# XuyangBai/D3Feat

Measured on AMD Instinct MI355X. Metric: fragments/sec (30k-pt clouds), higher is better.
Workload: dtype f32; 1 GPU; SURVEY §8d config #2: synthetic 3DMatch room fragment, 300k raw pts -> grid subsample 0.03 m (~29k pts per cloud) -> self-pair -> 5-level pyramid -> full KPFCNN forward (random-init weights (reference initialiser, seed 42), 14.1M params)...; points_per_cloud=29369, fragments_per_gpu=2141, parallelism=fragment-dp1, fragments_per_replay=12, engine_fallbacks=0, engine_isolated_replays=0

## Files before the change

### d3feat_amd/_lib.py

```python
import ctypes as C
import os

_HERE = os.path.dirname(os.path.abspath(__file__))
LIB_PATH = os.environ.get("D3FEAT_AMD_LIB") or os.path.join(_HERE, "lib", "libd3feat_amd.so")

D3F_OK = 0
ERRORS = {-1: "HIP runtime / kernel launch failure", -2: "workspace too small", -3: "invalid argument"}
ST_EMPTY_ELEMENT, ST_NEG_CELL, ST_KEY_RANGE, ST_HIT_OVERFLOW, ST_OUT_OVERFLOW, ST_KEY_WIDTH = 1, 2, 4, 8, 16, 32
PAD_NUM_SUPPORTS = -2147483648
NEIGHBOR_CAP = 1024
MAX_BATCH = 255
TOPK_MAX = 8192
PAIRS_KMAX = 1024
REPEAT_COUNTS_MAX = 16
MATCH_KMAX = 8192
VALIDATION_NMAX = 1024
SCENES_MAX = 256
GRID_RESET_MAX = 8
VP_INDEX_RANGE, VP_COUNT_RANGE = 1, 2

_vp, _sz, _i, _f = C.c_void_p, C.c_size_t, C.c_int, C.c_float

SIGNATURES = {
    "d3f_version": (_i, []),
    "d3f_trace_marker": (_i, [_i, _vp]),
    "d3f_pack_status": (_i, [_vp, _vp, _i, _vp, _i, _vp, _i, _vp, _i, _vp, _i, _i, _i, _vp]),
    "d3f_grid_subsample_workspace_bytes": (_sz, [_i, _i, _i, _i]),
    "d3f_batch_grid_subsample": (_i, [_vp, _i, _vp, _i, _f, _vp, _i, _vp, _i, _vp, _vp, _vp, _vp, _vp, _vp, _sz, _vp]),
    "d3f_batch_grid_subsample_async": (_i, [_vp, _i, _vp, _i, _f, _vp, _i, _i, _i, _vp, _vp, _vp, _sz, _vp]),
    "d3f_batch_grid_subsample_async_inplace": (_i, [_vp, _i, _vp, _i, _f, _vp, _i, _i, _vp, _vp, _vp, _sz, _vp]),
    "d3f_stack_self_pair": (_i, [_vp, _i, _vp, _i, _vp, _vp, _vp, _vp]),
    "d3f_radius_neighbors_workspace_bytes": (_sz, [_i, _i, _i]),
    "d3f_batch_radius_neighbors": (_i, [_vp, _i, _vp, _i, _vp, _vp, _i, _f, _vp, _i, _i, _i, _vp, _vp, _sz, _vp]),
    "d3f_neighbor_grid_bytes": (_sz, [_i, _i]),
    "d3f_neighbor_grid_order_offset": (_sz, [_i, _i]),
    "d3f_neighbor_grid_build": (_i, [_vp, _i, _vp, _i, _f, _vp, _sz, _vp]),
    "d3f_neighbor_grid_boxed_form": (_i, [_i, _i]),
    "d3f_geometry_reset": (_i, [_vp, _i, _vp, _vp, _vp, _vp, _i, _vp]),
    "d3f_neighbor_grid_build_boxed": (_i, [_vp, _i, _vp, _i, _f, _vp, _vp, _sz, _vp]),
    "d3f_stack_self_pair_boxed": (_i, [_vp, _i, _vp, _i, _vp, _vp, _vp, _vp, _vp, _vp]),
    "d3f_batch_grid_subsample_async_boxed": (_i, [_vp, _vp, _i, _vp, _i, _f, _vp, _i, _i, _i, _vp, _vp, _vp, _vp, _vp, _sz, _vp]),
    "d3f_neighbor_grid_search": (_i, [_vp, _sz, _i, _vp, _i, _vp, _i, _f, _i, _vp, _i, _i, _i, _i, _i, _f, _i, _vp, _vp]),
    "d3f_neighbor_grid_search_ordered": (_i, [_vp, _sz, _i, _vp, _i, _vp, _i, _f, _vp, _sz, _vp, _i, _i, _i, _i, _i, _f, _i, _vp, _vp]),
    "d3f_neighbor_grid_inv_offset": (_sz, [_i, _i]),
    "d3f_neighbor_grid_xyz_offset": (_sz, [_i, _i]),
    "d3f_row_positive": (_i, [_vp, _i, _i, _i, _vp, _vp, _i, _vp]),
    "d3f_kpconv_aggregate": (_i, [_vp, _i, _vp, _i, _vp, _i, _i, _vp, _i, _i, _vp, _vp, _i, _f, _i, _i, _vp, _vp, _vp, _vp,
                                  _vp, _i, _vp]),
    "d3f_kpconv_deform_aggregate": (_i, [_vp, _i, _vp, _i, _vp, _i, _i, _vp, _i, _i, _vp, _i, _f, _vp, _i, _i, _vp, _i, _f, _i, _i, _vp,
                                         _vp, _vp, _vp, _i, _vp]),
    "d3f_kpconv_fused_c1": (_i, [_vp, _i, _vp, _i, _vp, _i, _i, _vp, _i, _vp, _i, _f, _i, _i, _vp, _i, _vp, _vp, _vp, _i, _i,
                                 _f, _vp, _i, _vp, _vp, _vp, _i, _vp]),
    "d3f_kpconv_fused32": (_i, [_vp, _i, _vp, _i, _vp, _i, _i, _vp, _i, _vp, _vp, _i, _f, _i, _i, _vp, _vp, _vp, _vp, _i, _i, _f, _vp,
                                _i, _vp, _vp, _vp, _i, _vp]),
    "d3f_kpconv_fused_supported": (_i, [_i, _i, _i, _i, _i]),
    "d3f_kpconv_pack_weights": (_i, [_vp, _i, _i, _vp, _vp]),
    "d3f_kpconv_fused": (_i, [_vp, _i, _vp, _i, _vp, _i, _i, _vp, _i, _i, _vp, _vp, _i, _f, _i, _i, _vp, _i, _vp, _vp, _vp, _i, _i,
                              _f, _vp, _i, _vp, _vp, _vp, _i, _vp]),
    "d3f_kpconv_fused32_x3": (_i, [_vp, _i, _vp, _i, _vp, _i, _i, _vp, _i, _vp, _vp, _i, _f, _i, _i, _vp, _vp, _vp, _vp, _i, _i, _f, _vp,
                                   _i, _vp, _vp, _vp, _i, _vp]),
    "d3f_kpconv_packed_x3_bytes": (_sz, [_i, _i]),
    "d3f_kpconv_pack_weights_x3": (_i, [_vp, _i, _i, _vp, _vp]),
    "d3f_kpconv_fused_x3": (_i, [_vp, _i, _vp, _i, _vp, _i, _i, _vp, _i, _i, _vp, _vp, _i, _f, _i, _i, _vp, _i, _vp, _vp, _vp, _i, _i,
                                 _f, _vp, _i, _vp, _vp, _vp, _i, _vp]),
    "d3f_gemm_workspace_bytes": (_sz, [_i, _i, _i, _i]),
    "d3f_gemm_bf16_workspace_bytes": (_sz, [_i, _i, _i, _i]),
    "d3f_gemm_f32": (_i, [_vp, _i, _vp, _i, _vp, _i, _i, _i, _i, _vp, _vp, _vp, _vp, _i, _i, _f, _vp, _sz, _vp, _i, _vp]),
    "d3f_gemm_upsample_cat_f32": (_i, [_vp, _i, _i, _i, _vp, _i, _vp, _i, _i, _vp, _i, _vp, _i, _i, _i, _vp, _vp, _i, _f, _vp, _sz,
                                       _vp, _vp, _i, _vp]),
    "d3f_ind_max_pool": (_i, [_vp, _i, _i, _i, _vp, _i, _i, _i, _vp, _i, _vp, _vp, _vp, _vp, _i, _vp]),
    "d3f_closest_pool_cat": (_i, [_vp, _i, _i, _i, _vp, _i, _i, _vp, _i, _i, _vp, _i, _vp, _vp, _vp]),
    "d3f_affine_act": (_i, [_vp, _i, _i, _i, _vp, _vp, _vp, _i, _i, _f, _vp, _i, _vp, _vp]),
    "d3f_pack_descriptors": (_i, [_vp, _vp, _i, _i, _vp, _i, _vp, _i, _vp, _vp]),
    "d3f_pack_descriptors_to": (_i, [_vp, _vp, _i, _i, _vp, _i, _vp, _i, _vp, _vp, _i, _i, _i, _vp, _vp, _vp]),
    "d3f_topk_workspace_bytes": (_sz, [_i, _i, _i, _i]),
    "d3f_topk_records": (_i, [_vp, _i, _vp, _i, _i, _vp, _i, _i, _vp, _vp, _i, _i, _i, _vp, _i, _i, _vp, _i, _vp, _vp, _vp, _vp, _sz,
                              _vp]),
    "d3f_feature_nn_workspace_bytes": (_sz, [_i]),
    "d3f_feature_nn": (_i, [_vp, _i, _i, _vp, _i, _i, _i, _vp, _vp, _vp, _sz, _vp]),
    "d3f_mutual_matches_workspace_bytes": (_sz, [_i]),
    "d3f_mutual_matches": (_i, [_vp, _i, _vp, _i, _vp, _vp, _vp, _sz, _vp]),
    "d3f_ransac_hypotheses": (_i, [_vp, _i, _vp, _i, _vp, _i, _f, _f, C.c_uint64, C.c_uint64, _i, _vp, _vp, _vp]),
    "d3f_ransac_draw": (_i, [C.c_uint64, C.c_uint64, _i, _i]),
    "d3f_neighbor_grid_score": (_i, [_vp, _sz, _i, _vp, _i, _vp, _i, _f, _vp, _vp, _vp, _vp]),
    "d3f_register_pairs_workspace_bytes": (_sz, [_i, _i, _i, _i]),
    "d3f_register_pairs": (_i, [_vp, _i, _i, _i, _i, _vp, _vp, _i, _i, _f, _i, _f, _f, _i, _i, C.c_uint64, _vp, _f] + [_vp] * 11
                           + [_sz, _vp]),
    "d3f_repeatability_pairs": (_i, [_vp, _i, _i, _i, _vp, _vp, _i, _vp, _i, _vp, _vp, _i, _vp, _vp, _vp]),
    "d3f_match_pairs_workspace_bytes": (_sz, [_i, _vp, _i]),
    "d3f_match_pairs": (_i, [_vp, _i, _i, _i, _i, _vp, _vp, _i, _vp, _f, _vp, _i, _vp, _vp, _vp, _sz, _vp]),
    "d3f_register_pairs_counts_workspace_bytes": (_sz, [_i, _i, _i, _vp, _i, _i]),
    "d3f_register_pairs_counts": (_i, [_vp, _i, _i, _i, _i, _vp, _vp, _i, _vp, _i, _f, _i, _f, _f, _i, _i, C.c_uint64, _vp, _f] + [_vp] * 10
                                  + [_sz, _vp]),
    "d3f_overlap_pairs": (_i, [_vp, _sz, _i, _i, _vp, _i, _f, _vp, _vp, _i, _vp]),
    "d3f_validation_pairs_workspace_bytes": (_sz, [_i, _i]),
    "d3f_validation_pairs": (_i, [_vp, _i, _i, _vp, _i, _vp, _i, _i, _vp, _vp, _vp, _i, _vp, _i, _f, _i, _f, _f, _f, _f] + [_vp] * 5
                             + [_sz, _vp]),
    "d3f_loss_gradients_workspace_bytes": (_sz, [_i, _i, _i]),
    "d3f_loss_gradients": (_i, [_vp, _i, _i, _vp, _i, _vp, _i, _i, _vp, _vp, _vp, _i, _vp, _i, _f, _i, _f, _f, _f, _f, _i, _vp, _i, _vp, _i,
                                _vp, _vp, _vp, _sz, _vp]),
    "d3f_neighbor_transpose_workspace_bytes": (_sz, [_i, _i]),
    "d3f_neighbor_transpose": (_i, [_vp, _i, _i, _i, _vp, _i, _vp, _vp, _vp, _sz, _vp]),
    "d3f_detect_head_backward_workspace_bytes": (_sz, [_i, _i, _i]),
    "d3f_detect_head_backward": (_i, [_vp, _i, _i, _i, _vp, _i, _i, _vp, _vp, _i, _i, _vp, _vp, _vp, _i, _vp, _i, _vp, _i, _vp, _sz, _vp]),
    "d3f_neighbor_transpose_qs": (_i, [_vp, _i, _i, _i, _vp, _i, _vp, _vp, _vp, _vp, _sz, _vp]),
    "d3f_kpconv_backward_workspace_bytes": (_sz, [_i, _i, _i, _i, _i, _i]),
    "d3f_kpconv_backward": (_i, [_vp, _i, _vp, _i, _vp, _i, _i, _vp, _i, _i, _vp, _i, _f, _i, _i, _vp, _vp, _i, _i, _vp, _vp, _vp, _i, _vp,
                                 _vp, _vp, _vp, _i, _vp, _sz, _vp]),
    "d3f_gemm_tn_workspace_bytes": (_sz, [_i, _i, _i]),
    "d3f_gemm_tn_f32": (_i, [_vp, _i, _vp, _i, _i, _i, _i, _vp, _vp, _vp, _sz, _vp]),
    "d3f_batch_norm_workspace_bytes": (_sz, [_i, _i]),
    "d3f_batch_norm_train": (_i, [_vp, _i, _i, _i, _vp, _vp, _f, _f, _vp, _vp, _vp, _i, _i, _f, _vp, _i, _vp, _vp, _vp, _vp, _sz, _vp]),
    "d3f_batch_norm_backward": (_i, [_vp, _i, _vp, _i, _vp, _i, _i, _i, _vp, _vp, _vp, _i, _f, _vp, _i, _vp, _vp, _vp, _i, _vp, _vp, _sz,
                                     _vp]),
    "d3f_pose_errors": (_i, [_vp, _vp, _i, _i, _vp, _vp, _vp, _vp, _vp, _vp]),
    "d3f_sanitize_descriptors": (_i, [_vp, _i, _i, _i, _i, _vp]),
    "d3f_matching_summary": (_i, [_vp, _vp, _vp, _i, _i, _vp, _i, _vp, _vp, _vp, _vp]),
    "d3f_registration_recall": (_i, [_vp, _i, _vp, _vp, _vp, _vp, _vp, _i, _i, _vp, _i, _vp, _vp, _vp, _vp, _vp]),
    "d3f_icp_pairs_workspace_bytes": (_sz, [_i, _i]),
    "d3f_icp_pairs": (_i, [_vp, _sz, _i, _vp, _i, _vp, _i, _vp, _vp, _i, _i] + [_vp] * 9 + [_sz, _vp]),
    "d3f_gemm_pack_bf16": (_i, [_vp, _i, _i, _i, _vp, _vp]),
    "d3f_gemm_pack_f32t": (_i, [_vp, _i, _i, _i, _vp, _vp]),
    "d3f_gemm_f32t": (_i, [_vp, _i, _i, _i, _vp, _i, _vp, _i, _i, _vp, _vp, _i, _i, _i, _vp, _vp, _vp, _vp, _i, _i, _f, _vp, _sz,
                           _vp, _vp, _i, _vp]),
    "d3f_gemm_x3_packed_bytes": (_sz, [_i, _i]),
    "d3f_gemm_pack_x3": (_i, [_vp, _i, _i, _i, _vp, _vp]),
    "d3f_gemm_x3_workspace_bytes": (_sz, [_i, _i, _i, _i]),
    "d3f_gemm_x3_plan": (_i, [_i, _i, _i, _i, _vp, _vp, _vp]),
    "d3f_gemm_x3_resident": (_i, [_i, _i, _i, _i]),
    "d3f_gemm_x3": (_i, [_vp, _i, _i, _i, _vp, _i, _vp, _i, _i, _vp, _vp, _i, _i, _i, _vp, _vp, _vp, _vp, _i, _i, _f, _vp, _sz,
                         _vp, _vp, _i, _vp]),
    "d3f_gemm_x3_gres": (_i, [_vp, _i, _i, _i, _vp, _i, _vp, _i, _i, _vp, _vp, _i, _i, _i, _vp, _vp, _vp, _vp, _i, _vp, _i, _i, _vp, _i, _f,
                              _vp, _sz, _vp, _vp, _i, _vp]),
    "d3f_gemm_pack_x3_chain": (_i, [_vp, _i, _i, _i, _vp, _vp]),
    "d3f_gemm_x3_chain_ok": (_i, [_i, _i, _i, _i, _i]),
    "d3f_gemm_x3_chain": (_i, [_vp, _i, _i, _i, _vp, _i, _vp, _i, _i, _vp, _vp, _i, _i, _i, _vp, _vp, _vp, _vp, _i, _i, _f, _vp,
                               _vp, _vp, _i, _f, _vp, _i, _vp, _vp, _vp]),
    "d3f_gemm_bf16": (_i, [_vp, _i, _i, _i, _vp, _i, _vp, _i, _i, _vp, _vp, _i, _i, _i, _vp, _vp, _vp, _vp, _i, _i, _f, _vp, _sz,
                           _vp, _vp, _i, _i, _i, _vp]),
    "d3f_decode_xyz_records": (_i, [_vp, _i, _i, _i, _i, _i, _i, _i, _vp, _vp]),
    "d3f_detect_head": (_i, [_vp, _i, _i, _i, _vp, _i, _i, _vp, _vp, _i, _i, _vp, _i, _vp, _vp, _vp, _vp]),
}

_lib = None


class D3FeatLibraryError(RuntimeError):
    pass


def load():
    global _lib
    if _lib is not None:
        return _lib
    if not os.path.exists(LIB_PATH):
        raise D3FeatLibraryError(
            "d3feat_amd: %s not found -- the HIP extension is the only compute path. Build it with "
            "`python -c 'import __graft_entry__ as g; g.build()'` or `make -C d3feat_amd/csrc`." % LIB_PATH)
    lib = C.CDLL(LIB_PATH)
    for name, (res, args) in SIGNATURES.items():
        fn = getattr(lib, name)
        fn.restype = res
        fn.argtypes = args
    _lib = lib
    return lib


def check(rc, what):
    if rc != D3F_OK:
        raise D3FeatLibraryError("d3feat_amd.%s failed: %s (code %d)" % (what, ERRORS.get(rc, "unknown"), rc))
```

### d3feat_amd/csrc/grid_subsample.hip

```cpp
#include <cstdlib>
#include "prims.h"
#include "radix_sort.h"

#define GS_EMPTY 0xFFFFFFFFFFFFFFFFull
#define GS_KEYBITS 56
#define GS_KEYMASK ((1ull << GS_KEYBITS) - 1ull)
#define GS_MAX_PROBE 4096

__constant__ unsigned long long D3F_CHAIN_DEV[D3F_NCHAIN] = {
    13ull, 29ull, 59ull, 127ull, 257ull, 541ull, 1109ull, 2357ull, 5087ull, 10273ull, 20753ull, 42043ull, 85229ull,
    172933ull, 351061ull, 712697ull, 1447153ull, 2938679ull, 5967347ull, 12117689ull, 24607243ull, 49969847ull,
    101473717ull, 206062531ull, 418451333ull, 849749479ull, 1725587117ull, 3504151727ull};

struct GsElem {
    float org[3];
    int pad0;
    unsigned long long NX, NY, NZ;
    long long bbase;
};

#include "gs_order.h"

__device__ __forceinline__ float gs_axis(unsigned mn, unsigned mx, float dl, float inv, float& org) {
    org = __fmul_rn(floorf(__fmul_rn(d3f_ord2f(mn), inv)), dl);
    return fmaxf(floorf(__fdiv_rn(__fsub_rn(d3f_ord2f(mx), org), dl)), 0.f);
}
__device__ __forceinline__ int gs_cell(const float* __restrict__ p, float ox, float oy, float oz, float dl, float& cx, float& cy,
                                       float& cz) {
    const float fx = floorf(__fdiv_rn(__fsub_rn(p[0], ox), dl));
    const float fy = floorf(__fdiv_rn(__fsub_rn(p[1], oy), dl));
    const float fz = floorf(__fdiv_rn(__fsub_rn(p[2], oz), dl));
    cx = fmaxf(fx, 0.f);
    cy = fmaxf(fy, 0.f);
    cz = fmaxf(fz, 0.f);
    return (fx < 0.f || fy < 0.f || fz < 0.f) ? D3F_ST_NEG_CELL : 0;
}

__device__ __forceinline__ float gs_inv_count(int c) { return (float)(1.0 / (double)c); }

__device__ __forceinline__ unsigned long long gs_mix(unsigned long long x) {
    x ^= x >> 33; x *= 0xff51afd7ed558ccdull; x ^= x >> 33; x *= 0xc4ceb9fe1a85ec53ull; x ^= x >> 33;
    return x;
}

__device__ __forceinline__ int gs_bits(unsigned long long x) {
    int b = 0;
    while (x) { ++b; x >>= 1; }
    return b;
}
__device__ __forceinline__ void gs_prep(const unsigned* __restrict__ bbox, const int* __restrict__ offs, int B, float dl,
                                        GsElem* __restrict__ el, int* __restrict__ status, RsMeta* __restrict__ smeta,
                                        int n_cap) {
    __shared__ unsigned long long sCells[256];
    const int b = threadIdx.x;
    unsigned long long cells = 0ull;
    if (b < B) {
        GsElem e;
        e.pad0 = 0;
        const int len = offs[b + 1] - offs[b];
        if (len <= 0) {
            atomicOr(&status[1], D3F_ST_EMPTY_ELEMENT);
            e.org[0] = e.org[1] = e.org[2] = 0.f;
            e.NX = e.NY = e.NZ = 1;
        } else {
            const float inv = __fdiv_rn(1.0f, dl);
            unsigned long long dims[3];
#pragma unroll
            for (int d = 0; d < 3; ++d) {
                const unsigned mn = __hip_atomic_load(&bbox[b * 6 + d], __ATOMIC_RELAXED, __HIP_MEMORY_SCOPE_AGENT);
                const unsigned mx = __hip_atomic_load(&bbox[b * 6 + 3 + d], __ATOMIC_RELAXED, __HIP_MEMORY_SCOPE_AGENT);
                dims[d] = (unsigned long long)gs_axis(mn, mx, dl, inv, e.org[d]) + 1ull;
            }
            e.NX = dims[0]; e.NY = dims[1]; e.NZ = dims[2];
        }
        long long base = 0;
        for (int j = 0; j < b; ++j) {
            long long l = offs[j + 1] - offs[j];
            unsigned long long nb = D3F_CHAIN_DEV[D3F_NCHAIN - 1];
            for (int c = 0; c < D3F_NCHAIN; ++c)
                if ((long long)D3F_CHAIN_DEV[c] >= l) { nb = D3F_CHAIN_DEV[c]; break; }
            base += (long long)nb;
        }
        e.bbase = base;
        el[b] = e;
        const double c = (double)e.NX * (double)e.NY * (double)e.NZ;
        cells = c >= 1.8e19 ? 0xFFFFFFFFFFFFFFFFull : e.NX * e.NY * e.NZ;
    }
    if (!smeta) return;
    sCells[threadIdx.x] = cells;
    __syncthreads();
    if (threadIdx.x == 0) {
        unsigned long long mx = 1ull;
        for (int j = 0; j < B; ++j) mx = sCells[j] > mx ? sCells[j] : mx;
        int kb = gs_bits(mx - 1ull);
        if (kb < 1) kb = 1;
        const int eb = gs_bits((unsigned long long)(B - 1));
        RsMeta m;
        m.n = min(offs[B], n_cap);
        m.kb = kb;
        m.bits = kb + eb;
        if (m.bits > 32) {
            atomicOr(&status[1], D3F_ST_KEY_WIDTH);
            m.n = 0;
            m.bits = 8;
        }
        m.npass = (m.bits + 7) / 8;
        *smeta = m;
    }
}
struct GsPrepEpi {
    const unsigned* bbox; const int* offs; int B; float dl; GsElem* el; int* status; RsMeta* smeta; int n_cap;
    __device__ __forceinline__ void operator()() const { gs_prep(bbox, offs, B, dl, el, status, smeta, n_cap); }
};

__global__ void __launch_bounds__(256) gs_begin_boxed_kernel(const int* __restrict__ lens, int B, int* __restrict__ offs,
                                                             const unsigned* __restrict__ bbox, unsigned* __restrict__ counters,
                                                             int ncounters, D3fFill f0, D3fFill fmeta, float dl, GsElem* __restrict__ el,
                                                             int* __restrict__ status, RsMeta* __restrict__ smeta, int n_cap) {
    const size_t tid = (size_t)blockIdx.x * blockDim.x + threadIdx.x, stride = (size_t)gridDim.x * blockDim.x;
    d3f_fill_words(f0, tid, stride);
    if (blockIdx.x != 0) return;
    if (threadIdx.x == 0) {
        int s = 0;
        for (int b = 0; b < B; ++b) { offs[b] = s; s += lens[b]; }
        offs[B] = s;
    }
    for (int i = threadIdx.x; i < ncounters; i += blockDim.x) counters[i] = 0u;
    for (int i = threadIdx.x; i < (int)fmeta.n; i += blockDim.x) fmeta.p[i] = fmeta.v;
    asm volatile("s_waitcnt vmcnt(0)" ::: "memory");
    __syncthreads();
    gs_prep(bbox, offs, B, dl, el, status, smeta, n_cap);
}

__global__ void __launch_bounds__(256) gs_insert_kernel(const float* __restrict__ pts, int N, const int* __restrict__ offs,
                                                        int B, float dl, const GsElem* __restrict__ el,
                                                        unsigned long long* __restrict__ tkey, unsigned* __restrict__ tfirst,
                                                        unsigned long long capmask, int* __restrict__ slot,
                                                        int* __restrict__ status) {
    const int i = blockIdx.x * blockDim.x + threadIdx.x;
    if (i >= min(N, offs[B])) return;
    const int b = d3f_find_elem(offs, B, i);
    const GsElem e = el[b];
    float cx, cy, cz;
    int st = gs_cell(pts + 3 * (size_t)i, e.org[0], e.org[1], e.org[2], dl, cx, cy, cz);
    const unsigned long long ix = (unsigned long long)cx, iy = (unsigned long long)cy, iz = (unsigned long long)cz;
    const unsigned long long key = ix + e.NX * iy + e.NX * e.NY * iz;
    if (key > GS_KEYMASK) st |= D3F_ST_KEY_RANGE;
    if (st) atomicOr(&status[1], st);
    const unsigned long long word = ((unsigned long long)b << GS_KEYBITS) | (key & GS_KEYMASK);
    unsigned long long h = gs_mix(word) & capmask;
    bool placed = false;
    for (int probe = 0; probe < GS_MAX_PROBE; ++probe) {
        unsigned long long prev = atomicCAS(&tkey[h], GS_EMPTY, word);
        if (prev == GS_EMPTY || prev == word) { placed = true; break; }
        h = (h + 1) & capmask;
    }
    if (!placed) atomicOr(&status[1], D3F_ST_OUT_OVERFLOW);
    atomicMin(&tfirst[h], (unsigned)i);
    slot[i] = (int)h;
}

struct GsMarkIn {
    const int* n_dev; const int* slot; const unsigned* tfirst;
    __device__ __forceinline__ int operator()(int i) const { return (i < *n_dev && tfirst[slot[i]] == (unsigned)i) ? 1 : 0; }
};

__global__ void __launch_bounds__(256) gs_chain_kernel(int N, const int* __restrict__ slot, const unsigned* __restrict__ tfirst,
                                                       const unsigned long long* __restrict__ tkey,
                                                       const int* __restrict__ vscan, const int* __restrict__ vbase,
                                                       int* __restrict__ pvid,
                                                       unsigned long long* __restrict__ vkey, int* __restrict__ vhead,
                                                       int* __restrict__ vcnt, int* __restrict__ pnext,
                                                       const int* __restrict__ n_dev) {
    const int i = blockIdx.x * blockDim.x + threadIdx.x;
    if (i >= min(N, *n_dev)) return;
    const int s = slot[i];
    const int fi = (int)tfirst[s];
    const int v = d3f_scan_at(vscan, vbase, fi);
    pvid[i] = v;
    if (fi == i) vkey[v] = tkey[s] & GS_KEYMASK;
    pnext[i] = atomicExch(&vhead[v], i);
    atomicAdd(&vcnt[v], 1);
}

struct GsRankScan {
    const int* vscan; const int* vbase;
    __device__ __forceinline__ int operator()(int p) const { return d3f_scan_at(vscan, vbase, p); }
};
struct GsRankBits {
    const unsigned* fbits; const int* wscan; const int* wbase;
    __device__ __forceinline__ int operator()(int p) const {
        const int w = p >> 5;
        return d3f_scan_at(wscan, wbase, w) + __popc(fbits[w] & ((1u << (p & 31)) - 1u));
    }
};
template <class Rank>
struct GsMoffsEpi {
    const int* offs; int B; Rank rank; int* meta; int* moffs; int* sub_lens; int* status_dev;
    int out_cap;
    int elem_cap;
    __device__ __forceinline__ void operator()(int M) const {
        if (threadIdx.x != 0) return;
        meta[0] = M;
        const int N = offs[B];
        for (int b = 0; b <= B; ++b) moffs[b] = (b == B || offs[b] >= N) ? M : rank(offs[b]);
        bool over = M > out_cap ||
                    (__hip_atomic_load(&meta[1], __ATOMIC_RELAXED, __HIP_MEMORY_SCOPE_AGENT) & (D3F_ST_OUT_OVERFLOW | D3F_ST_KEY_WIDTH));
        for (int b = 0; b < B; ++b) over = over || (moffs[b + 1] - moffs[b] > elem_cap);
        if (over && !(__hip_atomic_load(&meta[1], __ATOMIC_RELAXED, __HIP_MEMORY_SCOPE_AGENT) & D3F_ST_KEY_WIDTH))
            atomicOr(&meta[1], D3F_ST_OUT_OVERFLOW);
        for (int b = 0; b < B; ++b) {
            const int l = over ? 0 : moffs[b + 1] - moffs[b];
            meta[2 + b] = l;
            sub_lens[b] = l;
        }
        if (status_dev) {
            status_dev[0] = over ? 0 : M;
            status_dev[1] = __hip_atomic_load(&meta[1], __ATOMIC_RELAXED, __HIP_MEMORY_SCOPE_AGENT);
        }
    }
};

__global__ void __launch_bounds__(256) gs_rank_kernel(int N, const int* __restrict__ n_dev, const int* __restrict__ pvid,
                                                      const int* __restrict__ vhead, const int* __restrict__ pnext,
                                                      const int* __restrict__ vstart, const int* __restrict__ sbase,
                                                      int* __restrict__ sorted) {
    const int i = blockIdx.x * blockDim.x + threadIdx.x;
    if (i >= min(N, *n_dev)) return;
    const int v = pvid[i];
    int r = 0;
    for (int j = vhead[v]; j >= 0; j = pnext[j]) r += (j < i) ? 1 : 0;
    sorted[d3f_scan_at(vstart, sbase, v) + r] = i;
}

#define GS_SMALL_LAST 6
#define GS_TILE 1024

struct GsOrderArgs {
    const unsigned long long* vkey;
    const int* moffs;
    const int* offs;
    const GsElem* el;
    int* P[2];
    int* nx[2];
    int* cd;
    int* bkt[2];
    int* bf[2];
    int* bc[2];
    int* bh[2];
    int* tsum;
    int* vpos;
    int max_m;
};

#define GS_SMALL_NB 1109
#define GS_SMALL_T 256
__global__ void __launch_bounds__(GS_SMALL_T) gs_order_small_kernel(GsOrderArgs A) {
    __shared__ int wsum[GS_SMALL_T / 64];
    __shared__ int sBF[GS_SMALL_NB], sBC[GS_SMALL_NB], sBH[GS_SMALL_NB], sNX[GS_SMALL_NB], sCD[GS_SMALL_NB], sBK[GS_SMALL_NB];
    __shared__ int sL[2][GS_SMALL_NB];
    __shared__ unsigned long long sKey[GS_SMALL_NB];
    const int b = blockIdx.x;
    const int tid = threadIdx.x;
    const int M = A.moffs[b + 1] - A.moffs[b];
    if (M <= 0) return;
    const unsigned long long* key = A.vkey + A.moffs[b];
    int* VP = A.vpos + A.moffs[b];
    const long long bbase = A.el[b].bbase;
    for (int t = tid; t < min(M, GS_SMALL_NB); t += GS_SMALL_T) sKey[t] = key[t];
    __syncthreads();
    GsOrderLds<unsigned long long> S;
    S.key = sKey; S.bf = sBF; S.bc = sBC; S.bh = sBH; S.nx = sNX; S.cd = sCD; S.bk = sBK; S.L0 = sL[0]; S.L1 = sL[1];
    S.wsum = wsum;
    int lo;
    const int* list;
    const bool done = gs_order_rounds_lds<GS_SMALL_T, unsigned long long, true>(
        S, M, GS_SMALL_LAST,
        [VP](int* Lb, int id, int dest) {
            Lb[dest] = id;
            VP[id] = dest;
        },
        lo, list);
    if (!done && GS_SMALL_LAST + 1 < D3F_NCHAIN) {
        const int j = GS_SMALL_LAST + 1;
        int* P = A.P[j & 1] + A.offs[b];
        for (int t = tid; t < lo; t += GS_SMALL_T) P[t] = list[t];
        const int nb = (int)D3F_CHAIN_DEV[j];
        for (int t = tid; t < nb; t += GS_SMALL_T) gs_bucket_reset(A.bf[j & 1] + bbase, A.bc[j & 1] + bbase, A.bh[j & 1] + bbase, t);
    }
}

__device__ __forceinline__ bool gs_round(const GsOrderArgs& A, int b, int j, int& M, int& lo, int& hi, int& nb, bool& last) {
    M = A.moffs[b + 1] - A.moffs[b];
    lo = (int)D3F_CHAIN_DEV[j - 1];
    if (M <= lo || M > A.max_m) return false;
    nb = (int)D3F_CHAIN_DEV[j];
    last = M <= nb;
    hi = last ? M : nb;
    return true;
}

__global__ void __launch_bounds__(256) gs_order_insert_kernel(GsOrderArgs A, int j) {
    const int b = blockIdx.y;
    int M, lo, hi, nb;
    bool last;
    if (!gs_round(A, b, j, M, lo, hi, nb, last)) return;
    const int t = blockIdx.x * 256 + threadIdx.x;
    if (t >= hi) return;
    const int o = A.offs[b];
    const long long bbase = A.el[b].bbase;
    const int id = (t < lo) ? A.P[j & 1][o + t] : t;
    const int bk = gs_mod(A.vkey[A.moffs[b] + id], (unsigned)nb, 1.0 / (double)nb);
    A.nx[j & 1][o + t] = gs_bucket_insert(A.bf[j & 1] + bbase, A.bc[j & 1] + bbase, A.bh[j & 1] + bbase, bk, t);
    A.bkt[j & 1][o + t] = bk;
}

__device__ __forceinline__ void gs_order_scan_sums(const GsOrderArgs& A, int j, int b, int* wsum) {
    int M, lo, hi, nb;
    bool last;
    if (!gs_round(A, b, j, M, lo, hi, nb, last)) return;
    int* ts = A.tsum + A.offs[b] / GS_TILE + b;
    const int ntiles = (hi + GS_TILE - 1) / GS_TILE;
    int carry = 0;
    for (int c0 = 0; c0 < ntiles; c0 += 256) {
        const int i = c0 + (int)threadIdx.x;
        const int v = (i < ntiles) ? __hip_atomic_load(&ts[i], __ATOMIC_RELAXED, __HIP_MEMORY_SCOPE_AGENT) : 0;
        int tot;
        const int e = d3f_block_excl_scan<256>(v, wsum, &tot);
        if (i < ntiles) ts[i] = carry + e;
        carry += tot;
    }
}

__global__ void __launch_bounds__(256) gs_order_scan_tiles_kernel(GsOrderArgs A, int j, int B, unsigned* __restrict__ counter) {
    __shared__ int wsum[4];
    const int b = blockIdx.y;
    int M, lo, hi, nb;
    bool last;
    const int tile = blockIdx.x;
    const bool active = gs_round(A, b, j, M, lo, hi, nb, last) && tile * GS_TILE < hi;
    if (!active) return;
    {
        const int o = A.offs[b];
        const long long bbase = A.el[b].bbase;
        const int tid = threadIdx.x;
        if (!last && j + 1 < D3F_NCHAIN) {
            const int nbn = (int)D3F_CHAIN_DEV[j + 1];
            const int stride = ((hi + GS_TILE - 1) / GS_TILE) * 256;
            for (int i = tile * 256 + tid; i < nbn; i += stride)
                gs_bucket_reset(A.bf[(j + 1) & 1] + bbase, A.bc[(j + 1) & 1] + bbase, A.bh[(j + 1) & 1] + bbase, i);
        }
        int c[4], s = 0;
#pragma unroll
        for (int k = 0; k < 4; ++k) {
            const int u = tile * GS_TILE + tid * 4 + k, t = hi - 1 - u;
            c[k] = 0;
            if (u < hi) {
                const int bk = A.bkt[j & 1][o + t];
                c[k] = (A.bf[j & 1][bbase + bk] == t) ? A.bc[j & 1][bbase + bk] : 0;
            }
            s += c[k];
        }
        int tot;
        int run = d3f_block_excl_scan<256>(s, wsum, &tot);
#pragma unroll
        for (int k = 0; k < 4; ++k) {
            const int u = tile * GS_TILE + tid * 4 + k;
            if (u < hi) A.cd[o + hi - 1 - u] = run;
            run += c[k];
        }
        if (tid == 0) A.tsum[o / GS_TILE + b + tile] = tot;
    }
    if (!d3f_last_block(counter + b, (unsigned)((hi + GS_TILE - 1) / GS_TILE))) return;
    gs_order_scan_sums(A, j, b, wsum);
}

__global__ void __launch_bounds__(256) gs_order_place_kernel(GsOrderArgs A, int j) {
    const int b = blockIdx.y;
    int M, lo, hi, nb;
    bool last;
    if (!gs_round(A, b, j, M, lo, hi, nb, last)) return;
    const int t = blockIdx.x * 256 + threadIdx.x;
    const int o = A.offs[b];
    const long long bbase = A.el[b].bbase;
    const bool next = !last && j + 1 < D3F_NCHAIN;
    const int nbn = next ? (int)D3F_CHAIN_DEV[j + 1] : 1;
    int id = -1, pos = -1;
    if (t < hi) {
        id = (t < lo) ? A.P[j & 1][o + t] : t;
        const int bk = A.bkt[j & 1][o + t];
        int r = 0;
        for (int q = A.bh[j & 1][bbase + bk]; q >= 0; q = A.nx[j & 1][o + q]) r += (q > t) ? 1 : 0;
        const int f = A.bf[j & 1][bbase + bk];
        const int dest = A.cd[o + f] + A.tsum[o / GS_TILE + b + (hi - 1 - f) / GS_TILE] + r;
        A.P[(j + 1) & 1][o + dest] = id;
        if (last) A.vpos[A.moffs[b] + id] = dest;
        pos = dest;
    } else if (next && t < min(M, nbn)) {
        id = pos = t;
    }
    if (next && id >= 0) {
        const int bk = gs_mod(A.vkey[A.moffs[b] + id], (unsigned)nbn, 1.0 / (double)nbn);
        A.nx[(j + 1) & 1][o + pos] =
            gs_bucket_insert(A.bf[(j + 1) & 1] + bbase, A.bc[(j + 1) & 1] + bbase, A.bh[(j + 1) & 1] + bbase, bk, pos);
        A.bkt[(j + 1) & 1][o + pos] = bk;
    }
}

#include "gs_small.h"

__global__ void __launch_bounds__(RS_THREADS) gs_sortkey_kernel(const float* __restrict__ pts, const float* const* __restrict__ ptrs,
                                                                const int* __restrict__ offs, int B,
                                                                float dl, const GsElem* __restrict__ el,
                                                                const RsMeta* __restrict__ smeta, unsigned* __restrict__ skey,
                                                                unsigned* __restrict__ hist, int* __restrict__ status) {
    __shared__ unsigned sHist[256];
    __shared__ int sOffs[D3F_MAX_BATCH + 1];
    __shared__ GsElem sEl[D3F_MAX_BATCH];
    __shared__ const float* sBase[D3F_MAX_BATCH];
    const int n = smeta->n, kb = smeta->kb;
    const int tile = blockIdx.x;
    if ((long long)tile * RS_TILE >= (long long)n) return;
    for (int t = threadIdx.x; t <= B; t += RS_THREADS) sOffs[t] = offs[t];
    for (int t = threadIdx.x; t < B; t += RS_THREADS) {
        sEl[t] = el[t];
        sBase[t] = ptrs ? ptrs[t] - 3 * (size_t)offs[t] : pts;
    }
    __syncthreads();
    const int w = threadIdx.x >> 6, lane = threadIdx.x & 63;
    const int base = tile * RS_TILE + w * RS_WAVE_ITEMS + lane;
    const int wlo = tile * RS_TILE + w * RS_WAVE_ITEMS, whi = min(wlo + RS_WAVE_ITEMS, n) - 1;
    int b0 = 0;
    while (b0 + 1 < B && wlo >= sOffs[b0 + 1]) ++b0;
    const bool one_cloud = (b0 + 1 >= B) || whi < sOffs[b0 + 1];
    unsigned key[RS_ROUNDS], vm = 0u;
    int st = 0;
#pragma unroll
    for (int r = 0; r < RS_ROUNDS; ++r) {
        const int i = base + r * 64;
        key[r] = 0u;
        if (i < n) {
            int b = b0;
            if (!one_cloud)
                while (b + 1 < B && i >= sOffs[b + 1]) ++b;
            const float ox = sEl[b].org[0], oy = sEl[b].org[1], oz = sEl[b].org[2];
            const unsigned NX = (unsigned)sEl[b].NX, NY = (unsigned)sEl[b].NY;
            const float* __restrict__ P = sBase[b];
            float cx, cy, cz;
            st |= gs_cell(P + 3 * (size_t)i, ox, oy, oz, dl, cx, cy, cz);
            const unsigned ix = (unsigned)cx, iy = (unsigned)cy, iz = (unsigned)cz;
            const unsigned k = ix + NX * (iy + NY * iz);
            key[r] = (kb < 32 ? ((unsigned)b << kb) : 0u) | (kb < 32 ? (k & ((1u << kb) - 1u)) : k);
            skey[i] = key[r];
            vm |= 1u << r;
        }
    }
    if (st) atomicOr(&status[1], st);
    rs_tile_histogram(key, vm, 0, sHist, hist + (size_t)tile * 256);
}

__global__ void __launch_bounds__(256) gs_heads_kernel(int N, const RsMeta* __restrict__ smeta, const unsigned* __restrict__ key0,
                                                       const unsigned* __restrict__ key1, const unsigned* __restrict__ val0,
                                                       const unsigned* __restrict__ val1, unsigned* __restrict__ fbits) {
    const int j = blockIdx.x * blockDim.x + threadIdx.x;
    if (j >= min(N, smeta->n)) return;
    const unsigned* __restrict__ ks = (smeta->npass & 1) ? key1 : key0;
    const unsigned* __restrict__ vs = (smeta->npass & 1) ? val1 : val0;
    const unsigned k = ks[j];
    if (j == 0 || ks[j - 1] != k) {
        const unsigned i = vs[j];
        atomicOr(&fbits[i >> 5], 1u << (i & 31u));
    }
}
struct GsBitsIn {
    const unsigned* fbits;
    __device__ __forceinline__ int operator()(int w) const { return __popc(fbits[w]); }
};
__global__ void __launch_bounds__(256) gs_runs_kernel(int N, const RsMeta* __restrict__ smeta, const unsigned* __restrict__ key0,
                                                      const unsigned* __restrict__ key1, const unsigned* __restrict__ val0,
                                                      const unsigned* __restrict__ val1, GsRankBits rank,
                                                      const float* __restrict__ pts, const float* const* __restrict__ ptrs,
                                                      const int* __restrict__ offs, unsigned long long* __restrict__ vkey,
                                                      float* __restrict__ bary) {
    __shared__ float sx[256], sy[256], sz[256];
    __shared__ unsigned sk[256];
    const int n = min(N, smeta->n);
    const int j0 = blockIdx.x * 256;
    if (j0 >= n) return;
    const int t = threadIdx.x, j = j0 + t;
    const unsigned* __restrict__ ks = (smeta->npass & 1) ? key1 : key0;
    const unsigned* __restrict__ vs = (smeta->npass & 1) ? val1 : val0;
    unsigned k = 0u, pi = 0u, kprev = 0u;
    float px = 0.f, py = 0.f, pz = 0.f;
    if (j < n) {
        k = ks[j];
        pi = vs[j];
        kprev = j > 0 ? ks[j - 1] : 0u;
        if (ptrs) {
            const int b = smeta->kb < 32 ? (int)(k >> smeta->kb) : 0;
            pts = ptrs[b] - 3 * (size_t)offs[b];
        }
        px = pts[3 * (size_t)pi + 0]; py = pts[3 * (size_t)pi + 1]; pz = pts[3 * (size_t)pi + 2];
    }
    sx[t] = px; sy[t] = py; sz[t] = pz;
    sk[t] = k;
    __syncthreads();
    if (j >= n || (j != 0 && kprev == k)) return;
    const int v = rank((int)pi);
    float ax = px, ay = py, az = pz;
    int c = 1;
    const int lim = min(256, n - j0);
    while (t + c < lim && sk[t + c] == k) {
        ax = __fadd_rn(ax, sx[t + c]);
        ay = __fadd_rn(ay, sy[t + c]);
        az = __fadd_rn(az, sz[t + c]);
        ++c;
    }
    if (t + c == 256) {
        while (j + c < n && ks[j + c] == k) {
            const size_t q = vs[j + c];
            ax = __fadd_rn(ax, pts[3 * q + 0]);
            ay = __fadd_rn(ay, pts[3 * q + 1]);
            az = __fadd_rn(az, pts[3 * q + 2]);
            ++c;
        }
    }
    const float sc = gs_inv_count(c);
    vkey[v] = (unsigned long long)(smeta->kb < 32 ? (k & ((1u << smeta->kb) - 1u)) : k);
    bary[3 * (size_t)v + 0] = __fmul_rn(ax, sc);
    bary[3 * (size_t)v + 1] = __fmul_rn(ay, sc);
    bary[3 * (size_t)v + 2] = __fmul_rn(az, sc);
}
template <bool BOX>
__global__ void __launch_bounds__(BOX ? 1024 : 256) gs_emit_kernel(int* __restrict__ status, const int* __restrict__ moffs, int B,
                                                      const int* __restrict__ vpos, const float* __restrict__ bary,
                                                      float* __restrict__ out_p, int out_cap, unsigned* __restrict__ bbox_out) {
    const int v = blockIdx.x * blockDim.x + threadIdx.x;
    bool ok = v < status[0] && !(status[1] & (D3F_ST_OUT_OVERFLOW | D3F_ST_KEY_WIDTH));
    int b = -1;
    float x = 0.f, y = 0.f, z = 0.f;
    if (ok) {
        b = d3f_find_elem(moffs, B, v);
        const size_t dest = (size_t)moffs[b] + (size_t)vpos[v];
        if (dest >= (size_t)out_cap) {
            atomicOr(&status[1], D3F_ST_OUT_OVERFLOW);
            ok = false;
        } else {
            x = bary[3 * (size_t)v + 0]; y = bary[3 * (size_t)v + 1]; z = bary[3 * (size_t)v + 2];
            out_p[3 * dest + 0] = x;
            out_p[3 * dest + 1] = y;
            out_p[3 * dest + 2] = z;
        }
    }
    if constexpr (BOX) d3f_box_accum_block(bbox_out, ok ? b : -1, x, y, z);
}


__global__ void __launch_bounds__(256) gs_accum_kernel(const float* __restrict__ pts, const float* __restrict__ feat,
                                                       int fdim, int* __restrict__ status,
                                                       const int* __restrict__ moffs, int B,
                                                       const int* __restrict__ vstart, const int* __restrict__ sbase,
                                                       const int* __restrict__ vcnt,
                                                       const int* __restrict__ sorted, const int* __restrict__ vpos,
                                                       float* __restrict__ out_p, float* __restrict__ out_f, int out_cap) {
    const int v = blockIdx.x * blockDim.x + threadIdx.x;
    if (v >= status[0]) return;
    const int b = d3f_find_elem(moffs, B, v);
    const int n = vcnt[v], st = sbase ? d3f_scan_at(vstart, sbase, v) : vstart[v];
    const size_t dest = (size_t)moffs[b] + (size_t)vpos[v];
    if (dest >= (size_t)out_cap) {
        atomicOr(&status[1], D3F_ST_OUT_OVERFLOW);
        return;
    }
    float sx = 0.f, sy = 0.f, sz = 0.f;
    for (int t = 0; t < n; ++t) {
        const size_t i = (size_t)sorted[st + t];
        sx = __fadd_rn(sx, pts[3 * i + 0]);
        sy = __fadd_rn(sy, pts[3 * i + 1]);
        sz = __fadd_rn(sz, pts[3 * i + 2]);
    }
    const float sc = gs_inv_count(n);
    out_p[3 * dest + 0] = __fmul_rn(sx, sc);
    out_p[3 * dest + 1] = __fmul_rn(sy, sc);
    out_p[3 * dest + 2] = __fmul_rn(sz, sc);
    if (fdim > 0) {
        const float cf = (float)n;
        for (int f = 0; f < fdim; ++f) {
            float s = 0.f;
            for (int t = 0; t < n; ++t) s = __fadd_rn(s, feat[(size_t)sorted[st + t] * fdim + f]);
            out_f[dest * fdim + f] = __fdiv_rn(s, cf);
        }
    }
}

__global__ void __launch_bounds__(256) gs_labels_kernel(int N, int ldim, const int* __restrict__ cls,
                                                        const int* __restrict__ pvid, const int* __restrict__ moffs, int B,
                                                        const int* __restrict__ vpos, int* __restrict__ out_c) {
    const int i = blockIdx.x * blockDim.x + threadIdx.x;
    if (i >= N) return;
    const int v = pvid[i];
    const int b = d3f_find_elem(moffs, B, v);
    const size_t dest = (size_t)moffs[b] + (size_t)vpos[v];
    for (int l = 0; l < ldim; ++l) atomicMax(&out_c[dest * ldim + l], cls[(size_t)i * ldim + l]);
}

struct GsLayout {
    size_t cap;
    long long bucket_total;
};
static GsLayout gs_layout(int N, int B, int keys = -1) {
    GsLayout L;
    L.cap = 64;
    const size_t nk = (size_t)((keys > 0 && keys < N) ? keys : (N > 0 ? N : 1));
    while (L.cap < (size_t)2 * nk) L.cap <<= 1;
    L.bucket_total = (long long)(2.24 * (double)N) + 16ll * B + 64;
    return L;
}

extern "C" size_t d3f_grid_subsample_workspace_bytes(int N, int B, int fdim, int ldim) {
    (void)fdim; (void)ldim;
    if (N < 0 || B < 1) return 0;
    GsLayout L = gs_layout(N, B);
    size_t n = (size_t)(N > 0 ? N : 1);
    size_t bytes = 0;
    bytes += d3f_align((B + 1) * sizeof(int)) * 2 + d3f_align((B + 2) * sizeof(int));
    bytes += d3f_align(B * 6 * sizeof(unsigned));
    bytes += d3f_align(B * sizeof(GsElem));
    bytes += d3f_align(L.cap * sizeof(unsigned long long));
    bytes += d3f_align(L.cap * sizeof(int));
    bytes += d3f_align(n * sizeof(unsigned long long));
    bytes += 16 * d3f_align(n * sizeof(int));
    bytes += 6 * d3f_align((size_t)L.bucket_total * sizeof(int));
    bytes += d3f_align((n / GS_TILE + B + 8) * sizeof(int));
    bytes += 2 * d3f_align(d3f_scan_base_ints(N) * sizeof(int)) + d3f_align((4 + D3F_NCHAIN * (size_t)B) * sizeof(unsigned));
    bytes += d3f_align(rs_hist_words(N) * sizeof(unsigned)) + d3f_align((n / 32 + 2) * sizeof(unsigned)) +
             d3f_align(3 * n * sizeof(float)) + d3f_align(sizeof(RsMeta));
    bytes += d3f_align(7 * (size_t)B * (n < 16384 ? n : 16384) * sizeof(float)) + 256 + 2 * d3f_align(B * sizeof(int));
    return bytes + 4096;
}

template <int T, int R>
static int gs_small_launch(const GsSmallArgs& A, float* sub_points, int* sub_lens_dev, int* status_dev, hipStream_t stream) {
    static std::atomic<unsigned long long> lds_done{0ull};
    const void* const fns[] = {(const void*)gs_small_kernel<T, R>};
    if (d3f_opt_in_lds(lds_done, fns, (int)gss_lds_bytes<T, R>(GSS_NB_MAX)) != D3F_OK) return D3F_ERR_HIP;
    gs_small_kernel<T, R><<<A.B, T, gss_lds_bytes<T, R>(A.nbmax), stream>>>(A);
    D3F_LAUNCH_CHECK();
    gs_small_pack_kernel<<<d3f_cdiv(A.out_cap, 256), 256, 0, stream>>>(A, sub_points, sub_lens_dev, status_dev);
    D3F_LAUNCH_CHECK();
    return D3F_OK;
}
static int gs_run_small(const float* points, int N, const int* lens_dev, int B, float dl, float* sub_points, int M_cap, int elem_cap,
                        int pc, int* sub_lens_dev, int* status_dev, void* workspace, size_t workspace_bytes, hipStream_t stream,
                        unsigned* bbox_out = nullptr) {
    if (elem_cap <= 0 || elem_cap > M_cap) elem_cap = M_cap;
    if (elem_cap > pc) elem_cap = pc;
    D3fArena ar(workspace, workspace_bytes);
    GsSmallArgs A;
    A.stage = ar.take<float>(3 * (size_t)B * (size_t)elem_cap);
    A.recs = ar.take<float>(4 * (size_t)B * (size_t)elem_cap);
    A.mcount = ar.take<int>(B);
    A.cflags = ar.take<int>(B);
    if (!ar.ok) return D3F_ERR_WORKSPACE;
    A.bbox_out = bbox_out;
    A.pts = points; A.lens = lens_dev; A.B = B; A.dl = dl; A.elem_cap = elem_cap; A.pc = pc; A.out_cap = M_cap;
    A.nbmax = GSS_NB_MAX;
    for (int j = 0; j < D3F_NCHAIN; ++j)
        if ((long long)D3F_CHAIN_HOST[j] >= (long long)elem_cap) { A.nbmax = (int)D3F_CHAIN_HOST[j]; break; }
    if (A.nbmax > GSS_NB_MAX) A.nbmax = GSS_NB_MAX;
    if (A.nbmax < 1109) A.nbmax = 1109;
    if (pc <= 2048) return gs_small_launch<256, 8>(A, sub_points, sub_lens_dev, status_dev, stream);
    if (pc <= 4096) return gs_small_launch<512, 8>(A, sub_points, sub_lens_dev, status_dev, stream);
    if (pc <= 8192) return gs_small_launch<1024, 8>(A, sub_points, sub_lens_dev, status_dev, stream);
    if (pc <= 12288) return gs_small_launch<1024, 12>(A, sub_points, sub_lens_dev, status_dev, stream);
    return gs_small_launch<1024, 16>(A, sub_points, sub_lens_dev, status_dev, stream);
}

struct GsCall {
    const float* points; int N; const int* lens_dev; int B; float dl;
    const float* features; int fdim; const int* classes; int ldim;
    float* sub_points; int M_cap; float* sub_features; int* sub_classes; int* sub_lens_dev;
    int* status_host;
    int* status_dev;
    hipStream_t stream;
    const float* const* ptrs;
    const unsigned* bbox_in;
    unsigned* bbox_out;
};

struct GsWork {
    GsLayout L;
    int *offs, *moffs;
    unsigned* bbox;
    GsElem* el;
    int ncounters;
    unsigned* counters;
    unsigned long long* tkey;
    unsigned* tfirst;
    int* vhead;
    int* meta;
    int* vcnt;
    unsigned long long* vkey;
    int *slot, *vscan, *pvid, *pnext, *vstart, *sorted;
    GsOrderArgs A;
    int* vbase;
    int* sbase;
    unsigned* rs_hist;
    unsigned* fbits;
    float* bary;
    RsMeta* smeta;

    bool carve(void* workspace, size_t workspace_bytes, int N, int B, int keys) {
        L = gs_layout(N, B, keys);
        D3fArena ar(workspace, workspace_bytes);
        const size_t n = (size_t)N;
        offs = ar.take<int>(B + 1);
        moffs = ar.take<int>(B + 1);
        bbox = ar.take<unsigned>(B * 6);
        el = ar.take<GsElem>(B);
        ncounters = 4 + D3F_NCHAIN * B;
        counters = ar.take<unsigned>(ncounters);
        tkey = ar.take<unsigned long long>(L.cap);
        tfirst = ar.take<unsigned>(L.cap);
        vhead = ar.take<int>(n);
        meta = ar.take<int>(B + 2);
        vcnt = ar.take<int>(n);
        vkey = ar.take<unsigned long long>(n);
        slot = ar.take<int>(n);
        vscan = ar.take<int>(n);
        pvid = ar.take<int>(n);
        pnext = ar.take<int>(n);
        vstart = ar.take<int>(n);
        sorted = ar.take<int>(n);
        A.vpos = ar.take<int>(n);
        A.P[0] = ar.take<int>(n);
        A.P[1] = ar.take<int>(n);
        A.nx[0] = ar.take<int>(n);
        A.nx[1] = ar.take<int>(n);
        A.cd = ar.take<int>(n);
        A.bkt[0] = ar.take<int>(n);
        A.bkt[1] = ar.take<int>(n);
        for (int k = 0; k < 2; ++k) {
            A.bf[k] = ar.take<int>((size_t)L.bucket_total);
            A.bc[k] = ar.take<int>((size_t)L.bucket_total);
            A.bh[k] = ar.take<int>((size_t)L.bucket_total);
        }
        A.tsum = ar.take<int>(n / GS_TILE + B + 8);
        vbase = ar.take<int>(d3f_scan_base_ints(N));
        sbase = ar.take<int>(d3f_scan_base_ints(N));
        rs_hist = ar.take<unsigned>(rs_hist_words(N));
        fbits = ar.take<unsigned>(n / 32 + 2);
        bary = ar.take<float>(3 * n);
        smeta = ar.take<RsMeta>(1);
        A.vkey = vkey; A.moffs = moffs; A.offs = offs; A.el = el;
        return ar.ok;
    }
};

static int gs_order_launch(const GsWork& W, int B, int maxM, hipStream_t stream) {
    gs_order_small_kernel<<<B, GS_SMALL_T, 0, stream>>>(W.A);
    for (int j = GS_SMALL_LAST + 1; j < D3F_NCHAIN && (long long)D3F_CHAIN_HOST[j - 1] < (long long)maxM; ++j) {
        const long long nbj = (long long)D3F_CHAIN_HOST[j];
        const int hi = (int)((long long)maxM < nbj ? (long long)maxM : nbj);
        const bool more = j + 1 < D3F_NCHAIN && nbj < (long long)maxM;
        const long long nbn = more ? (long long)D3F_CHAIN_HOST[j + 1] : 0;
        const int hin = more ? (int)((long long)maxM < nbn ? (long long)maxM : nbn) : hi;
        dim3 g(d3f_cdiv(hi, 256), B), gt(d3f_cdiv(hi, GS_TILE), B), gp(d3f_cdiv(hin > hi ? hin : hi, 256), B);
        if (j == GS_SMALL_LAST + 1) gs_order_insert_kernel<<<g, 256, 0, stream>>>(W.A, j);
        gs_order_scan_tiles_kernel<<<gt, 256, 0, stream>>>(W.A, j, B, W.counters + 4 + j * B);
        gs_order_place_kernel<<<gp, 256, 0, stream>>>(W.A, j);
    }
    D3F_LAUNCH_CHECK();
    return D3F_OK;
}

static int gs_run_sort(const GsCall& C, const GsWork& W, int elem_cap) {
    const int N = C.N, B = C.B;
    const size_t n = (size_t)N;
    hipStream_t stream = C.stream;
    int rc;
    const D3fFill none{nullptr, 0ull, 0u};
    const D3fFill fill_bits{W.fbits, (unsigned long long)(n / 32 + 2), 0u};
    const D3fFill fill_meta{(unsigned*)W.meta, (unsigned long long)(B + 2), 0u};
    if (C.bbox_in) {
        long long blocks = (long long)(fill_bits.n / 4 / 256) + 1;
        if (blocks > 1024) blocks = 1024;
        gs_begin_boxed_kernel<<<(int)blocks, 256, 0, stream>>>(C.lens_dev, B, W.offs, C.bbox_in, W.counters, W.ncounters, fill_bits,
                                                               fill_meta, C.dl, W.el, W.meta, W.smeta, N);
        D3F_LAUNCH_CHECK();
    } else {
        if ((rc = d3f_begin_launch(C.lens_dev, B, W.offs, W.bbox, W.counters, W.ncounters, fill_bits, fill_meta, none, none,
                                   stream)) != D3F_OK)
            return rc;
        GsPrepEpi prep{W.bbox, W.offs, B, C.dl, W.el, W.meta, W.smeta, N};
        if ((rc = d3f_bbox_launch_t(C.points, W.offs, B, N, W.bbox, W.counters, prep, stream, C.ptrs)) != D3F_OK) return rc;
    }
    const int nblk = d3f_cdiv(N, 256);
    unsigned *key0 = (unsigned*)W.slot, *key1 = (unsigned*)W.pnext, *val0 = (unsigned*)W.pvid, *val1 = (unsigned*)W.sorted;
    gs_sortkey_kernel<<<rs_tiles(N), RS_THREADS, 0, stream>>>(C.points, C.ptrs, W.offs, B, C.dl, W.el, W.smeta, key0, W.rs_hist,
                                                              W.meta);
    D3F_LAUNCH_CHECK();
    if ((rc = rs_sort_launch(W.smeta, N, key0, key1, val0, val1, W.rs_hist, stream)) != D3F_OK) return rc;
    gs_heads_kernel<<<nblk, 256, 0, stream>>>(N, W.smeta, key0, key1, val0, val1, W.fbits);
    D3F_LAUNCH_CHECK();
    const GsRankBits rank{W.fbits, W.vscan, W.vbase};
    GsMoffsEpi<GsRankBits> mepi{W.offs, B, rank, W.meta, W.moffs, C.sub_lens_dev, C.status_dev, C.M_cap, elem_cap};
    if ((rc = d3f_scan_fold_launch(GsBitsIn{W.fbits}, N / 32 + 1, nullptr, W.vscan, W.vbase, W.counters + 1, mepi, stream)) != D3F_OK)
        return rc;
    gs_runs_kernel<<<nblk, 256, 0, stream>>>(N, W.smeta, key0, key1, val0, val1, rank, C.points, C.ptrs, W.offs, W.vkey, W.bary);
    D3F_LAUNCH_CHECK();
    const int M = N < C.M_cap ? N : C.M_cap;
    if ((rc = gs_order_launch(W, B, elem_cap, stream)) != D3F_OK) return rc;
    if (C.bbox_out)
        gs_emit_kernel<true><<<d3f_cdiv(M, 1024), 1024, 0, stream>>>(W.meta, W.moffs, B, W.A.vpos, W.bary, C.sub_points, C.M_cap,
                                                                     C.bbox_out);
    else
        gs_emit_kernel<false><<<d3f_cdiv(M, 256), 256, 0, stream>>>(W.meta, W.moffs, B, W.A.vpos, W.bary, C.sub_points, C.M_cap,
                                                                    nullptr);
    D3F_LAUNCH_CHECK();
    return D3F_OK;
}

static int gs_run_hash(const GsCall& C, const GsWork& W, int elem_cap) {
    const int N = C.N, B = C.B;
    const size_t n = (size_t)N;
    const bool async = C.status_dev != nullptr;
    hipStream_t stream = C.stream;
    int rc;
    const D3fFill none{nullptr, 0ull, 0u};
    const unsigned long long ones_words = (unsigned long long)((char*)(W.vhead + n) - (char*)W.tkey) / 4ull;
    const unsigned long long zero_words = (unsigned long long)((char*)(W.vcnt + n) - (char*)W.meta) / 4ull;
    if ((rc = d3f_begin_launch(C.lens_dev, B, W.offs, W.bbox, W.counters, W.ncounters, D3fFill{(unsigned*)W.tkey, ones_words, 0xFFFFFFFFu},
                               D3fFill{(unsigned*)W.meta, zero_words, 0u}, none, none, stream)) != D3F_OK)
        return rc;
    GsPrepEpi prep{W.bbox, W.offs, B, C.dl, W.el, W.meta, nullptr, N};
    if ((rc = d3f_bbox_launch_t(C.points, W.offs, B, N, W.bbox, W.counters, prep, stream, C.ptrs)) != D3F_OK) return rc;
    const int nblk = d3f_cdiv(N, 256);
    GsMoffsEpi<GsRankScan> mepi{W.offs, B, GsRankScan{W.vscan, W.vbase}, W.meta, W.moffs, C.sub_lens_dev, C.status_dev, C.M_cap,
                                async ? elem_cap : 0x7fffffff};
    gs_insert_kernel<<<nblk, 256, 0, stream>>>(C.points, N, W.offs, B, C.dl, W.el, W.tkey, W.tfirst, (unsigned long long)W.L.cap - 1ull,
                                               W.slot, W.meta);
    D3F_LAUNCH_CHECK();
    if ((rc = d3f_scan_fold_launch(GsMarkIn{W.offs + B, W.slot, W.tfirst}, N, W.offs + B, W.vscan, W.vbase, W.counters + 1, mepi,
                                   stream)) != D3F_OK)
        return rc;
    int M, maxM;
    if (!async) {
        D3F_HIP_TRY(hipMemcpyAsync(C.status_host, W.meta, (B + 2) * sizeof(int), hipMemcpyDeviceToHost, stream));
        D3F_HIP_TRY(hipStreamSynchronize(stream));
        M = C.status_host[0];
        if (C.status_host[1] != 0 || M <= 0) return D3F_OK;
        maxM = 0;
        for (int b = 0; b < B; ++b) maxM = C.status_host[2 + b] > maxM ? C.status_host[2 + b] : maxM;
    } else {
        M = N < C.M_cap ? N : C.M_cap;
        maxM = elem_cap;
    }
    gs_chain_kernel<<<nblk, 256, 0, stream>>>(N, W.slot, W.tfirst, W.tkey, W.vscan, W.vbase, W.pvid, W.vkey, W.vhead, W.vcnt, W.pnext,
                                              W.offs + B);
    D3F_LAUNCH_CHECK();
    if ((rc = d3f_scan_fold_launch(D3fScanIn{W.vcnt}, async ? N : M, W.meta, W.vstart, W.sbase, W.counters + 2, D3fNoEpi{},
                                   stream)) != D3F_OK)
        return rc;
    gs_rank_kernel<<<nblk, 256, 0, stream>>>(N, W.offs + B, W.pvid, W.vhead, W.pnext, W.vstart, W.sbase, W.sorted);
    if ((rc = gs_order_launch(W, B, maxM, stream)) != D3F_OK) return rc;
    gs_accum_kernel<<<d3f_cdiv(async ? N : M, 256), 256, 0, stream>>>(C.points, C.features, C.fdim, W.meta, W.moffs, B, W.vstart,
                                                                     W.sbase, W.vcnt, W.sorted, W.A.vpos, C.sub_points,
                                                                     C.sub_features, C.M_cap);
    D3F_LAUNCH_CHECK();
    if (C.ldim > 0) {
        if ((rc = d3f_fill_u32(C.sub_classes, (size_t)M * (size_t)C.ldim, 0x80000000u, stream)) != D3F_OK) return rc;
        gs_labels_kernel<<<nblk, 256, 0, stream>>>(N, C.ldim, C.classes, W.pvid, W.moffs, B, W.A.vpos, C.sub_classes);
        D3F_LAUNCH_CHECK();
    }
    return D3F_OK;
}

static int gs_run(const GsCall& C, int elem_cap, int elem_points, void* workspace, size_t workspace_bytes) {
    const bool async = C.status_dev != nullptr;
    const bool use_sort = async && !C.features && C.ldim == 0;
    if (use_sort && !C.ptrs) {
        const int pc = (elem_points > 0 && elem_points < C.N) ? elem_points : C.N;
        int ec = (elem_cap > 0 && elem_cap < C.M_cap) ? elem_cap : C.M_cap;
        if (ec > pc) ec = pc;
        if (pc <= 16384 && ec <= GSS_NB_MAX)
            return gs_run_small(C.points, C.N, C.lens_dev, C.B, C.dl, C.sub_points, C.M_cap, elem_cap, pc, C.sub_lens_dev, C.status_dev,
                                workspace, workspace_bytes, C.stream, C.bbox_out);
    }
    GsWork W;
    if (!W.carve(workspace, workspace_bytes, C.N, C.B, async ? C.M_cap : -1)) return D3F_ERR_WORKSPACE;
    if (elem_cap <= 0 || elem_cap > C.M_cap) elem_cap = C.M_cap;
    if (elem_cap > C.N) elem_cap = C.N;
    W.A.max_m = async ? elem_cap : 0x7fffffff;
    return use_sort ? gs_run_sort(C, W, elem_cap) : gs_run_hash(C, W, elem_cap);
}

extern "C" int d3f_batch_grid_subsample(const float* points, int N, const int* lens_dev, int B, float dl,
                                        const float* features, int fdim, const int* classes, int ldim,
                                        float* sub_points, float* sub_features, int* sub_classes, int* sub_lens_dev,
                                        int* status_host, void* workspace, size_t workspace_bytes, void* stream_) {
    hipStream_t stream = (hipStream_t)stream_;
    if (N < 0 || N > (1 << 30) || B < 1 || B > D3F_MAX_BATCH || !(dl > 0.f) || fdim < 0 || ldim < 0) return D3F_ERR_ARG;
    if (!points || !lens_dev || !sub_points || !sub_lens_dev || !status_host) return D3F_ERR_ARG;
    if ((fdim > 0 && (!features || !sub_features)) || (ldim > 0 && (!classes || !sub_classes))) return D3F_ERR_ARG;
    for (int i = 0; i < B + 2; ++i) status_host[i] = 0;
    if (N == 0) return d3f_fill_u32(sub_lens_dev, B, 0u, stream);
    const GsCall C{points, N, lens_dev, B, dl, features, fdim, classes, ldim, sub_points, N, sub_features, sub_classes, sub_lens_dev,
                   status_host, nullptr, stream, nullptr, nullptr, nullptr};
    return gs_run(C, N, 0, workspace, workspace_bytes);
}

extern "C" int d3f_batch_grid_subsample_async_boxed(const float* points, const float* const* clouds_dev, int N_cap, const int* lens_dev,
                                                    int B, float dl, float* sub_points, int M_cap, int elem_cap, int elem_points_cap,
                                                    int* sub_lens_dev, int* status_dev, const unsigned* bbox_in_dev,
                                                    unsigned* bbox_out_dev, void* workspace, size_t workspace_bytes, void* stream_) {
    if (N_cap < 1 || N_cap > (1 << 30) || M_cap < 1 || elem_cap < 0 || elem_points_cap < 0 || B < 1 || B > D3F_MAX_BATCH || !(dl > 0.f))
        return D3F_ERR_ARG;
    if ((!points && !clouds_dev) || (points && clouds_dev) || !lens_dev || !sub_points || !sub_lens_dev || !status_dev) return D3F_ERR_ARG;
    const GsCall C{points, N_cap, lens_dev, B, dl, nullptr, 0, nullptr, 0, sub_points, M_cap, nullptr, nullptr, sub_lens_dev,
                   nullptr, status_dev, (hipStream_t)stream_, clouds_dev, bbox_in_dev, bbox_out_dev};
    return gs_run(C, elem_cap, clouds_dev ? 0 : elem_points_cap, workspace, workspace_bytes);
}
extern "C" int d3f_batch_grid_subsample_async(const float* points, int N_cap, const int* lens_dev, int B, float dl,
                                              float* sub_points, int M_cap, int elem_cap, int elem_points_cap, int* sub_lens_dev,
                                              int* status_dev, void* workspace, size_t workspace_bytes, void* stream_) {
    return d3f_batch_grid_subsample_async_boxed(points, nullptr, N_cap, lens_dev, B, dl, sub_points, M_cap, elem_cap, elem_points_cap,
                                                sub_lens_dev, status_dev, nullptr, nullptr, workspace, workspace_bytes, stream_);
}
extern "C" int d3f_batch_grid_subsample_async_inplace(const float* const* clouds_dev, int N_cap, const int* lens_dev, int B, float dl,
                                                      float* sub_points, int M_cap, int elem_cap, int* sub_lens_dev, int* status_dev,
                                                      void* workspace, size_t workspace_bytes, void* stream_) {
    return d3f_batch_grid_subsample_async_boxed(nullptr, clouds_dev, N_cap, lens_dev, B, dl, sub_points, M_cap, elem_cap, 0, sub_lens_dev,
                                                status_dev, nullptr, nullptr, workspace, workspace_bytes, stream_);
}

__global__ void __launch_bounds__(256) gs_stack_pair_kernel(const float* __restrict__ pts, int M_cap, const int* __restrict__ lens_in,
                                                            int B, float* __restrict__ out, int* __restrict__ lens_out,
                                                            int* __restrict__ total, const unsigned* __restrict__ bbox_in,
                                                            unsigned* __restrict__ bbox_out) {
    const int i = blockIdx.x * blockDim.x + threadIdx.x;
    if (bbox_out && i < 12 * B) bbox_out[i] = bbox_in[(i / 12) * 6 + i % 6];
    int tot = 0;
    for (int b = 0; b < B; ++b) tot += lens_in[b];
    tot = min(tot, M_cap);
    if (i == 0) {
        int room = M_cap;
        for (int b = 0; b < B; ++b) {
            const int m = min(lens_in[b], room);
            room -= m;
            lens_out[2 * b] = m;
            lens_out[2 * b + 1] = m;
        }
        *total = 2 * tot;
    }
    if (i >= 3 * tot) return;
    const int pi = i / 3, c = i - 3 * pi;
    int start = 0, m = 0;
    for (int b = 0; b < B; ++b) {
        m = lens_in[b];
        if (pi < start + m || b == B - 1) break;
        start += m;
    }
    m = min(m, tot - start);
    const float v = pts[i];
    const size_t row = 2 * (size_t)start + (size_t)(pi - start);
    out[3 * row + c] = v;
    out[3 * (row + m) + c] = v;
}

extern "C" int d3f_stack_self_pair_boxed(const float* pts, int M_cap, const int* lens_in_dev, int B, float* out, int* lens_out_dev,
                                         int* total_dev, const unsigned* bbox_in_dev, unsigned* bbox_out_dev, void* stream_) {
    hipStream_t stream = (hipStream_t)stream_;
    if (M_cap < 1 || B < 1 || 2 * B > D3F_MAX_BATCH || !pts || !lens_in_dev || !out || !lens_out_dev || !total_dev ||
        (bbox_out_dev && !bbox_in_dev))
        return D3F_ERR_ARG;
    gs_stack_pair_kernel<<<d3f_cdiv(3ll * M_cap, 256), 256, 0, stream>>>(pts, M_cap, lens_in_dev, B, out, lens_out_dev, total_dev,
                                                                         bbox_in_dev, bbox_out_dev);
    D3F_LAUNCH_CHECK();
    return D3F_OK;
}
extern "C" int d3f_stack_self_pair(const float* pts, int M_cap, const int* lens_in_dev, int B, float* out, int* lens_out_dev,
                                   int* total_dev, void* stream_) {
    return d3f_stack_self_pair_boxed(pts, M_cap, lens_in_dev, B, out, lens_out_dev, total_dev, nullptr, nullptr, stream_);
}
```

### d3feat_amd/csrc/radix_sort.h

```cpp
#pragma once
#include "common.h"

#define RS_THREADS 512
#define RS_WAVES (RS_THREADS / 64)
#define RS_ROUNDS 16
#define RS_TILE (RS_THREADS * RS_ROUNDS)
#define RS_WAVE_ITEMS (64 * RS_ROUNDS)
#define RS_MAX_PASSES 4

struct RsMeta {
    int n;
    int bits;
    int npass;
    int kb;
};

#define RS_SCATTER_LDS_BYTES ((2 * RS_WAVES * 256 + 256 + 16 + 2 * RS_TILE) * 4)
static inline int rs_tiles(int n_cap) { return d3f_cdiv(n_cap > 0 ? n_cap : 1, RS_TILE); }
static inline size_t rs_hist_words(int n_cap) { return (size_t)rs_tiles(n_cap) * 256; }

#ifdef __HIPCC__
__device__ __forceinline__ void rs_tile_histogram(const unsigned (&key)[RS_ROUNDS], unsigned valid_mask, int shift,
                                                  unsigned* __restrict__ sHist, unsigned* __restrict__ hist_row) {
    if (threadIdx.x < 256) sHist[threadIdx.x] = 0u;
    __syncthreads();
#pragma unroll
    for (int r = 0; r < RS_ROUNDS; ++r)
        if (valid_mask & (1u << r)) atomicAdd(&sHist[(key[r] >> shift) & 255u], 1u);
    __syncthreads();
    if (threadIdx.x < 256) hist_row[threadIdx.x] = sHist[threadIdx.x];
}

template <int W>
__device__ __forceinline__ unsigned rs_wave_bases(unsigned (*sCnt)[256], unsigned* sScan) {
    const int tid = threadIdx.x, w = tid >> 6;
    unsigned cnt = 0u;
    if (tid < 256) {
#pragma unroll
        for (int q = 0; q < W; ++q) cnt += sCnt[q][tid];
    }
    const unsigned x = d3f_wave_incl_scan(cnt);
    if ((tid & 63) == 63) sScan[w] = x;
    __syncthreads();
    unsigned loc = 0u;
    if (tid < 256) {
        unsigned wb = 0u;
#pragma unroll
        for (int q = 0; q < 4; ++q) wb += (q < w) ? sScan[q] : 0u;
        loc = wb + x - cnt;
        unsigned run = loc;
#pragma unroll
        for (int q = 0; q < W; ++q) {
            const unsigned c = sCnt[q][tid];
            sCnt[q][tid] = run;
            run += c;
        }
    }
    return loc;
}

__global__ void __launch_bounds__(RS_THREADS) rs_hist_kernel(const RsMeta* __restrict__ meta, int pass,
                                                             const unsigned* __restrict__ key0,
                                                             const unsigned* __restrict__ key1,
                                                             unsigned* __restrict__ hist) {
    __shared__ unsigned sHist[256];
    const int n = meta->n;
    if (pass >= meta->npass) return;
    const int tile = blockIdx.x;
    if ((long long)tile * RS_TILE >= (long long)n) return;
    const unsigned* __restrict__ src = (pass & 1) ? key1 : key0;
    const int w = threadIdx.x >> 6, lane = threadIdx.x & 63;
    const int base = tile * RS_TILE + w * RS_WAVE_ITEMS + lane;
    unsigned key[RS_ROUNDS], vm = 0u;
#pragma unroll
    for (int r = 0; r < RS_ROUNDS; ++r) {
        const int pos = base + r * 64;
        key[r] = 0u;
        if (pos < n) { key[r] = src[pos]; vm |= 1u << r; }
    }
    rs_tile_histogram(key, vm, pass * 8, sHist, hist + (size_t)tile * 256);
}

__global__ void __launch_bounds__(RS_THREADS) rs_scatter_kernel(const RsMeta* __restrict__ meta, int pass,
                                                                unsigned* __restrict__ key0, unsigned* __restrict__ key1,
                                                                unsigned* __restrict__ val0, unsigned* __restrict__ val1,
                                                                const unsigned* __restrict__ hist) {
    extern __shared__ __attribute__((aligned(16))) unsigned rs_lds[];
    unsigned (*sCnt)[256] = (unsigned (*)[256])rs_lds;
    unsigned (*sPart)[256] = (unsigned (*)[256])(rs_lds + RS_WAVES * 256);
    unsigned* sBase = rs_lds + 2 * RS_WAVES * 256;
    unsigned* sScan = sBase + 256;
    unsigned* sKey = sScan + 16;
    unsigned* sVal = sKey + RS_TILE;
    const int n = meta->n;
    if (pass >= meta->npass) return;
    const int tile = blockIdx.x;
    if ((long long)tile * RS_TILE >= (long long)n) return;
    const int live = (n + RS_TILE - 1) / RS_TILE;
    const unsigned* __restrict__ ksrc = (pass & 1) ? key1 : key0;
    const unsigned* __restrict__ vsrc = (pass & 1) ? val1 : val0;
    unsigned* __restrict__ kdst = (pass & 1) ? key0 : key1;
    unsigned* __restrict__ vdst = (pass & 1) ? val0 : val1;
    const int tid = threadIdx.x, w = tid >> 6, lane = tid & 63;
    const int shift = pass * 8;

    const int base = tile * RS_TILE + w * RS_WAVE_ITEMS + lane;
    unsigned key[RS_ROUNDS], val[RS_ROUNDS];
#pragma unroll
    for (int r = 0; r < RS_ROUNDS; ++r) {
        const int pos = base + r * 64;
        key[r] = 0u;
        val[r] = (unsigned)pos;
        if (pos < n) {
            key[r] = ksrc[pos];
            if (pass > 0) val[r] = vsrc[pos];
        }
    }
    {
        uint4 bef = make_uint4(0u, 0u, 0u, 0u), tot = make_uint4(0u, 0u, 0u, 0u);
        const uint4* __restrict__ rows = (const uint4*)hist + lane;
        int t = w;
        for (; t + 7 * RS_WAVES < live; t += 8 * RS_WAVES) {
            uint4 v[8];
#pragma unroll
            for (int u = 0; u < 8; ++u) v[u] = rows[(size_t)(t + u * RS_WAVES) * 64];
#pragma unroll
            for (int u = 0; u < 8; ++u) {
                tot.x += v[u].x; tot.y += v[u].y; tot.z += v[u].z; tot.w += v[u].w;
                if (t + u * RS_WAVES < tile) { bef.x += v[u].x; bef.y += v[u].y; bef.z += v[u].z; bef.w += v[u].w; }
            }
        }
        for (; t < live; t += RS_WAVES) {
            const uint4 v = rows[(size_t)t * 64];
            tot.x += v.x; tot.y += v.y; tot.z += v.z; tot.w += v.w;
            if (t < tile) { bef.x += v.x; bef.y += v.y; bef.z += v.z; bef.w += v.w; }
        }
        ((uint4*)sCnt[w])[lane] = tot;
        ((uint4*)sPart[w])[lane] = bef;
    }
    __syncthreads();
    {
        unsigned total = 0u, before = 0u;
        if (tid < 256) {
#pragma unroll
            for (int q = 0; q < RS_WAVES; ++q) { total += sCnt[q][tid]; before += sPart[q][tid]; }
        }
        const unsigned x = d3f_wave_incl_scan(total);
        if (lane == 63) sScan[w] = x;
        __syncthreads();
#pragma unroll
        for (int q = 0; q < RS_WAVES; ++q)
            if (tid < 256) sCnt[q][tid] = 0u;
        unsigned wb = 0u;
#pragma unroll
        for (int q = 0; q < 4; ++q) wb += (q < w) ? sScan[q] : 0u;
        if (tid < 256) sBase[tid] = wb + x - total + before;
        __syncthreads();
    }
    unsigned rank[RS_ROUNDS];
    volatile unsigned* myCnt = sCnt[w];
#pragma unroll
    for (int r = 0; r < RS_ROUNDS; ++r) {
        const bool valid = (base + r * 64) < n;
        const unsigned dg = (key[r] >> shift) & 255u;
        unsigned long long peers = __ballot(valid);
#pragma unroll
        for (int bit = 0; bit < 8; ++bit) {
            const bool one = (dg >> bit) & 1u;
            const unsigned long long m = __ballot(one);
            peers &= one ? m : ~m;
        }
        rank[r] = 0u;
        if (valid) {
            const unsigned prev = myCnt[dg];
            const unsigned below = (unsigned)__popcll(peers & d3f_lanemask_lt());
            rank[r] = prev + below;
            __builtin_amdgcn_wave_barrier();
            if (below == 0u) myCnt[dg] = prev + (unsigned)__popcll(peers);
        }
        __builtin_amdgcn_wave_barrier();
    }
    __syncthreads();
    {
        const unsigned loc = rs_wave_bases<RS_WAVES>(sCnt, sScan);
        if (tid < 256) sBase[tid] -= loc;
    }
    __syncthreads();
#pragma unroll
    for (int r = 0; r < RS_ROUNDS; ++r) {
        if ((base + r * 64) < n) {
            const unsigned dg = (key[r] >> shift) & 255u;
            const unsigned pl = myCnt[dg] + rank[r];
            sKey[pl] = key[r];
            sVal[pl] = val[r];
        }
    }
    __syncthreads();
    const int tile_n = min(RS_TILE, n - tile * RS_TILE);
#pragma unroll
    for (int r = 0; r < RS_ROUNDS; ++r) {
        const int pl = r * RS_THREADS + tid;
        if (pl < tile_n) {
            const unsigned k = sKey[pl];
            const unsigned dest = sBase[(k >> shift) & 255u] + (unsigned)pl;
            kdst[dest] = k;
            vdst[dest] = sVal[pl];
        }
    }
}
#endif

static inline int rs_sort_launch(const RsMeta* meta, int n_cap, unsigned* key0, unsigned* key1, unsigned* val0, unsigned* val1,
                                 unsigned* hist, hipStream_t stream) {
    const int tiles = rs_tiles(n_cap);
    static std::atomic<unsigned long long> lds_done{0ull};
    const void* const fns[] = {(const void*)rs_scatter_kernel};
    if (d3f_opt_in_lds(lds_done, fns, RS_SCATTER_LDS_BYTES) != D3F_OK) return D3F_ERR_HIP;
    for (int p = 0; p < RS_MAX_PASSES; ++p) {
        if (p > 0) {
            rs_hist_kernel<<<tiles, RS_THREADS, 0, stream>>>(meta, p, key0, key1, hist);
            D3F_LAUNCH_CHECK();
        }
        rs_scatter_kernel<<<tiles, RS_THREADS, RS_SCATTER_LDS_BYTES, stream>>>(meta, p, key0, key1, val0, val1, hist);
        D3F_LAUNCH_CHECK();
    }
    return D3F_OK;
}
```

### include/d3feat_amd.h

```cpp
#ifndef D3FEAT_AMD_H
#define D3FEAT_AMD_H

#include <stddef.h>
#include <stdint.h>

#ifdef __cplusplus
extern "C" {
#endif

#define D3F_OK 0
#define D3F_ERR_HIP (-1)
#define D3F_ERR_WORKSPACE (-2)
#define D3F_ERR_ARG (-3)

#define D3F_ST_EMPTY_ELEMENT 1
#define D3F_ST_NEG_CELL 2
#define D3F_ST_KEY_RANGE 4
#define D3F_ST_HIT_OVERFLOW 8
#define D3F_ST_OUT_OVERFLOW 16
#define D3F_ST_KEY_WIDTH 32

#define D3F_NB_NO_KMAX 2
#define D3F_PAD_NUM_SUPPORTS (-2147483647 - 1)

#define D3F_MAX_BATCH 255
#define D3F_NEIGHBOR_CAP 1024
#define D3F_TOPK_MAX 8192
#define D3F_PAIRS_KMAX 1024
#define D3F_REPEAT_COUNTS_MAX 16
#define D3F_SCENES_MAX 256
#define D3F_MATCH_KMAX 8192
#define D3F_VALIDATION_NMAX 1024
#define D3F_NUM_KP_MAX 16

int d3f_version(void);

int d3f_trace_marker(int id, void* stream);
int d3f_pack_status(int* dst, const int* a, int na, const int* b, int nb, const int* c, int nc, const int* d, int nd,
                    int* clear, int nclear, int clear_first, int clear_step, void* stream);


size_t d3f_grid_subsample_workspace_bytes(int N, int B, int fdim, int ldim);
int d3f_batch_grid_subsample_async(const float* points, int N_cap, const int* lens_dev, int B, float dl,
                                   float* sub_points, int M_cap, int elem_cap, int elem_points_cap, int* sub_lens_dev,
                                   int* status_dev, void* workspace, size_t workspace_bytes, void* stream);
int d3f_batch_grid_subsample_async_inplace(const float* const* clouds_dev, int N_cap, const int* lens_dev, int B, float dl,
                                           float* sub_points, int M_cap, int elem_cap, int* sub_lens_dev, int* status_dev,
                                           void* workspace, size_t workspace_bytes, void* stream);

int d3f_stack_self_pair(const float* pts, int M_cap, const int* lens_in_dev, int B, float* out, int* lens_out_dev,
                        int* total_dev, void* stream);
int d3f_stack_self_pair_boxed(const float* pts, int M_cap, const int* lens_in_dev, int B, float* out, int* lens_out_dev,
                              int* total_dev, const unsigned* bbox_in_dev, unsigned* bbox_out_dev, void* stream);
int d3f_batch_grid_subsample_async_boxed(const float* points, const float* const* clouds_dev, int N_cap, const int* lens_dev,
                                         int B, float dl, float* sub_points, int M_cap, int elem_cap, int elem_points_cap,
                                         int* sub_lens_dev, int* status_dev, const unsigned* bbox_in_dev,
                                         unsigned* bbox_out_dev, void* workspace, size_t workspace_bytes, void* stream);
int d3f_batch_grid_subsample(const float* points, int N, const int* lens_dev, int B, float dl,
                             const float* features, int fdim, const int* classes, int ldim,
                             float* sub_points, float* sub_features, int* sub_classes, int* sub_lens_dev,
                             int* status_host, void* workspace, size_t workspace_bytes, void* stream);

size_t d3f_radius_neighbors_workspace_bytes(int Nq, int Ns, int B);
int d3f_batch_radius_neighbors(const float* queries, int Nq, const float* supports, int Ns,
                               const int* q_lens_dev, const int* s_lens_dev, int B, float radius,
                               int* out, int ld, int width, int pad_value, int* status_dev,
                               void* workspace, size_t workspace_bytes, void* stream);

size_t d3f_neighbor_grid_bytes(int Ns, int B);
size_t d3f_neighbor_grid_order_offset(int Ns, int B);
int d3f_neighbor_grid_build(const float* supports, int Ns, const int* s_lens_dev, int B, float radius,
                            void* grid, size_t grid_bytes, void* stream);
#define D3F_GRID_RESET_MAX 8
int d3f_neighbor_grid_boxed_form(int Ns, int B);
int d3f_geometry_reset(unsigned* boxes_dev, int n_boxes, const void* const* grids, const size_t* grid_bytes, const int* Ns,
                       const int* B, int n_grids, void* stream);
int d3f_neighbor_grid_build_boxed(const float* supports, int Ns, const int* s_lens_dev, int B, float radius,
                                  const unsigned* bbox_dev, void* grid, size_t grid_bytes, void* stream);
int d3f_neighbor_grid_search(const void* grid, size_t grid_bytes, int Ns, const float* queries, int Nq,
                             const int* q_lens_dev, int B, float radius, int queries_are_supports,
                             int* out, int ld, int width, int pad_value, int cap, int first_only, float nn_hint,
                             int reset_status, int* status_dev, void* stream);
#define D3F_NB_INTERNAL 4
int d3f_neighbor_grid_search_ordered(const void* grid, size_t grid_bytes, int Ns, const float* queries, int Nq,
                                     const int* q_lens_dev, int B, float radius, const void* query_grid, size_t query_grid_bytes,
                                     int* out, int ld, int width, int pad_value, int cap, int first_only, float nn_hint, int flags,
                                     int* status_dev, void* stream);
size_t d3f_neighbor_grid_inv_offset(int Ns, int B);
size_t d3f_neighbor_grid_xyz_offset(int Ns, int B);



int d3f_row_positive(const void* f, int Ns, int ldf, int Cin, unsigned char* row_pos, const int* Ns_dev, int feat_bf16,
                     void* stream);
int d3f_kpconv_aggregate(const float* q, int Nq, const float* s, int Ns, const int* idx, int ld_idx, int K,
                         const void* f, int ldf, int Cin, const unsigned char* row_pos, const float* kp_host,
                         int num_kp, float KP_extent, int influence, int aggregation, float* wf, float* inv_cnt,
                         const int* Nq_dev, const int* Ns_dev, const int* q_order, int feat_bf16, void* stream);

int d3f_kpconv_deform_aggregate(const float* q, int Nq, const float* s, int Ns, const int* idx, int ld_idx, int K,
                                const void* f, int ldf, int Cin, const float* offsets, int ld_off, float offset_scale,
                                const float* modulations, int ld_mod, int mod_logits, const float* kp_host, int num_kp,
                                float KP_extent, int influence, int aggregation, float* wf, const int* Nq_dev, const int* Ns_dev,
                                const int* q_order, int feat_bf16, void* stream);

int d3f_kpconv_fused_c1(const float* q, int Nq, const float* s, int Ns, const int* idx, int ld_idx, int K,
                        const float* f, int ldf, const float* kp_host, int num_kp, float KP_extent, int influence,
                        int aggregation, const float* W, int Cout, const float* col_scale, const float* col_shift,
                        const float* residual, int ldr, int leaky, float alpha, void* out, int ldo,
                        const int* Nq_dev, const int* Ns_dev, const int* q_order, int out_bf16, void* stream);

int d3f_kpconv_fused32(const float* q, int Nq, const float* s, int Ns, const int* idx, int ld_idx, int K,
                       const void* f, int ldf, const unsigned char* row_pos, const float* kp_host, int num_kp,
                       float KP_extent, int influence, int aggregation, const float* W, const float* col_scale,
                       const float* col_shift, const float* residual, int ldr, int leaky, float alpha, void* out, int ldo,
                       const int* Nq_dev, const int* Ns_dev, const int* q_order, int feat_bf16, void* stream);

int d3f_kpconv_fused_supported(int Cin, int Cout, int num_kp, int influence, int aggregation);
int d3f_kpconv_pack_weights(const float* W, int K, int N, float* W_packed, void* stream);
size_t d3f_kpconv_packed_x3_bytes(int K, int N);
int d3f_kpconv_pack_weights_x3(const float* W, int K, int N, void* W_planes, void* stream);
int d3f_kpconv_fused32_x3(const float* q, int Nq, const float* s, int Ns, const int* idx, int ld_idx, int K,
                          const void* f, int ldf, const unsigned char* rowpos, const float* kp_host, int num_kp,
                          float KP_extent, int influence, int aggregation, const float* W_planes, const float* col_scale,
                          const float* col_shift, const float* residual, int ldr, int leaky, float alpha, void* out,
                          int ldo, const int* Nq_dev, const int* Ns_dev, const int* q_order, int feat_bf16, void* stream);
int d3f_kpconv_fused_x3(const float* q, int Nq, const float* s, int Ns, const int* idx, int ld_idx, int K,
                        const void* f, int ldf, int Cin, const unsigned char* rowpos, const float* kp_host, int num_kp,
                        float KP_extent, int influence, int aggregation, const float* W_planes, int Cout,
                        const float* col_scale, const float* col_shift, const float* residual, int ldr, int leaky,
                        float alpha, void* out, int ldo, const int* Nq_dev, const int* Ns_dev, const int* q_order,
                        int feat_bf16, void* stream);
int d3f_kpconv_fused(const float* q, int Nq, const float* s, int Ns, const int* idx, int ld_idx, int K,
                     const void* f, int ldf, int Cin, const unsigned char* rowpos, const float* kp_host, int num_kp,
                     float KP_extent, int influence, int aggregation, const float* W_packed, int Cout,
                     const float* col_scale, const float* col_shift, const float* residual, int ldr, int leaky,
                     float alpha, void* out, int ldo, const int* Nq_dev, const int* Ns_dev, const int* q_order,
                     int feat_bf16, void* stream);

size_t d3f_gemm_workspace_bytes(int M, int N, int K, int M_hint);
int d3f_gemm_f32(const float* A, int lda, const float* B, int ldb, float* C, int ldc, int M, int N, int K,
                 const float* row_scale, const float* col_scale, const float* col_shift,
                 const float* residual, int ldr, int leaky, float alpha,
                 void* workspace, size_t workspace_bytes, const int* M_dev, int M_hint, void* stream);

int d3f_gemm_upsample_cat_f32(const float* x, int N1, int ldx, int C1, const int* idx, int ld_idx,
                              const float* skip, int lds, int C2, const float* W, int ldb, float* C, int ldc,
                              int M, int N, const float* col_scale, const float* col_shift, int leaky, float alpha,
                              void* workspace, size_t workspace_bytes, const int* M_dev, const int* N1_dev,
                              int M_hint, void* stream);

int d3f_ind_max_pool(const void* x, int N1, int ldx, int C, const int* idx, int N2, int ld_idx, int K,
                     void* out, int ldo, float* col_min_dev, const int* N1_dev, const int* N2_dev, const int* row_order,
                     int feat_bf16, void* stream);
int d3f_closest_pool_cat(const float* x, int N1, int ldx, int C1, const int* idx, int N2, int ld_idx,
                         const float* skip, int lds, int C2, float* out, int ldo, const int* N1_dev, const int* N2_dev,
                         void* stream);

int d3f_affine_act(const float* x, int ldx, int M, int N, const float* col_scale, const float* col_shift,
                   const float* residual, int ldr, int leaky, float alpha, float* out, int ldo, const int* M_dev,
                   void* stream);

int d3f_detect_head(const float* x, int N, int ldx, int C, const int* idx, int ld_idx, int K,
                    const int* lens_dev, const int* include_zero_dev, int stack_group, int B, float* desc, int ldd,
                    float* score, int* scratch_dev, const int* row_order, void* stream);

int d3f_pack_descriptors(const float* xyz, const float* desc, int ldd, int C, const float* score, int N, float* out,
                         int ldo, const int* N_dev, void* stream);
int d3f_pack_descriptors_to(const float* xyz, const float* desc, int ldd, int C, const float* score, int N, float* out,
                            int ldo, const int* N_dev, const int* lens_dev, int B, int group, int keep,
                            const long long* dst_ptrs_dev, const int* row_map_dev, void* stream);

size_t d3f_topk_workspace_bytes(int N, int B, int n_cap, int K);
int d3f_topk_records(const float* xyz, int ldx, const float* desc, int ldd, int C, const float* score, int lds, int N,
                     const int* N_dev, const int* lens_dev, int B, int group, int keep, const int* row_map_dev, int n_cap, int K,
                     float* out, int ldo, int* idx_out, int* count_dev, int* tickets_dev, void* workspace, size_t workspace_bytes,
                     void* stream);

int d3f_gemm_pack_f32t(const float* W, int ldb, int K, int N, float* Wt, void* stream);
int d3f_gemm_f32t(const float* A, int N1, int lda, int C1, const int* idx, int ld_idx, const float* skip, int lds, int C2,
                  const float* Wt, float* C, int ldc, int M, int N, const float* row_scale, const float* col_scale,
                  const float* col_shift, const float* residual, int ldr, int leaky, float alpha, void* workspace,
                  size_t workspace_bytes, const int* M_dev, const int* N1_dev, int M_hint, void* stream);

size_t d3f_gemm_x3_packed_bytes(int K, int N);
int d3f_gemm_pack_x3(const float* W, int ldb, int K, int N, void* Wx, void* stream);
size_t d3f_gemm_x3_workspace_bytes(int M, int N, int K, int M_hint);
int d3f_gemm_x3_plan(int M, int N, int K, int M_hint, int* rows, int* cols, int* slices);
int d3f_gemm_x3_resident(int M, int N, int K, int M_hint);
int d3f_gemm_x3(const float* A, int N1, int lda, int C1, const int* idx, int ld_idx, const float* skip, int lds, int C2,
                const void* Wx, float* C, int ldc, int M, int N, const float* row_scale, const float* col_scale,
                const float* col_shift, const float* residual, int ldr, int leaky, float alpha, void* workspace,
                size_t workspace_bytes, const int* M_dev, const int* N1_dev, int M_hint, void* stream);
int d3f_gemm_x3_gres(const float* A, int N1, int lda, int C1, const int* idx, int ld_idx, const float* skip, int lds, int C2,
                     const void* Wx, float* C, int ldc, int M, int N, const float* row_scale, const float* col_scale,
                     const float* col_shift, const float* residual, int ldr, const int* res_idx, int ld_res_idx, int res_rows,
                     const int* res_rows_dev, int leaky, float alpha, void* workspace, size_t workspace_bytes, const int* M_dev,
                     const int* N1_dev, int M_hint, void* stream);

int d3f_gemm_pack_x3_chain(const float* W2, int ldb, int K, int N, void* W2x, void* stream);
int d3f_gemm_x3_chain_ok(int M, int N, int K, int store_first, int M_hint);
int d3f_gemm_x3_chain(const float* A, int N1, int lda, int C1, const int* idx, int ld_idx, const float* skip, int lds, int C2cols,
                      const void* Wx, float* C, int ldc, int M, int N, const float* row_scale, const float* col_scale,
                      const float* col_shift, const float* residual, int ldr, int leaky, float alpha, const void* W2x,
                      const float* col_scale2, const float* col_shift2, int leaky2, float alpha2, float* C2, int ldc2,
                      const int* M_dev, const int* N1_dev, void* stream);

size_t d3f_gemm_bf16_workspace_bytes(int M, int N, int K, int M_hint);
int d3f_gemm_pack_bf16(const float* W, int ldb, int K, int N, void* W_packed, void* stream);
int d3f_gemm_bf16(const void* A, int N1, int lda, int C1, const int* idx, int ld_idx, const void* skip, int lds, int C2,
                  const void* W_packed, void* C, int ldc, int M, int N, const float* row_scale, const float* col_scale,
                  const float* col_shift, const void* residual, int ldr, int leaky, float alpha, void* workspace,
                  size_t workspace_bytes, const int* M_dev, const int* N1_dev, int M_hint, int a_bf16, int c_bf16, void* stream);

int d3f_decode_xyz_records(const void* raw, int n, int stride, int off_x, int off_y, int off_z, int is_f64, int big_endian,
                           float* out, void* stream);


size_t d3f_feature_nn_workspace_bytes(int Na);
int d3f_feature_nn(const float* A, int Na, int lda, const float* B, int Nb, int ldb, int C, int* idx, float* d2_out,
                   void* workspace, size_t workspace_bytes, void* stream);

size_t d3f_mutual_matches_workspace_bytes(int Na);
int d3f_mutual_matches(const int* ab, int Na, const int* ba, int Nb, int* pairs, int* count_dev, void* workspace,
                       size_t workspace_bytes, void* stream);

int d3f_ransac_hypotheses(const float* src, int Ns, const float* tgt, int Nt, const int* nn, int ransac_n,
                          float edge_similarity, float checker_distance, uint64_t seed, uint64_t it0,
                          int H, float* T_out, unsigned char* valid_out, void* stream);
int d3f_ransac_draw(uint64_t seed, uint64_t iteration, int d, int n);

int d3f_neighbor_grid_score(const void* grid, size_t grid_bytes, int Nt, const float* src, int Ns, const float* T, int V,
                            float radius, int* count_dev, uint64_t* sumd2_dev, int* nearest_dev, void* stream);

size_t d3f_register_pairs_workspace_bytes(int P, int K, int num_keypts, int max_validation);
int d3f_register_pairs(const float* kp, int n_blocks, int K, int ld, int C, const int* count_dev, const int* pairs_dev, int P,
                       int num_keypts, float max_correspondence_distance, int ransac_n, float edge_similarity,
                       float checker_distance, int max_iteration, int max_validation, uint64_t seed, const float* gt,
                       float distance_threshold, float* T_out, int* inliers, uint64_t* sumd2, int* validations, int* iterations,
                       int* best_iteration, int* mutual_count, int* nearest, int* mutual, int* gt_inliers, void* workspace,
                       size_t workspace_bytes, void* stream);

int d3f_repeatability_pairs(const float* kp, int n_blocks, int K, int ld, const int* count_dev, const int* pairs_dev, int P,
                            const double* gt_dev, int moved, const double* threshold_host, const int* num_keypts_host,
                            int n_counts, int* repeat_dev, int64_t* totals_dev, void* stream);

size_t d3f_match_pairs_workspace_bytes(int P, const int* num_keypts_host, int n_counts);
int d3f_match_pairs(const float* kp, int n_blocks, int K, int ld, int C, const int* count_dev, const int* pairs_dev, int P,
                    const float* gt, float distance_threshold, const int* num_keypts_host, int n_counts, int* mutual_count,
                    int* gt_inliers, void* workspace, size_t workspace_bytes, void* stream);

size_t d3f_register_pairs_counts_workspace_bytes(int P, int n_blocks, int K, const int* num_keypts_host, int n_counts,
                                                 int max_validation);
int d3f_register_pairs_counts(const float* kp, int n_blocks, int K, int ld, int C, const int* count_dev, const int* pairs_dev, int P,
                              const int* num_keypts_host, int n_counts, float max_correspondence_distance, int ransac_n,
                              float edge_similarity, float checker_distance, int max_iteration, int max_validation, uint64_t seed,
                              const float* gt, float distance_threshold, float* T_out, int* inliers, uint64_t* sumd2,
                              int* validations, int* iterations, int* best_iteration, int* mutual_count, int* gt_inliers,
                              int* nearest, void* workspace, size_t workspace_bytes, void* stream);

int d3f_overlap_pairs(const void* grid, size_t grid_bytes, int N, int B, const int* pairs_dev, int P, float threshold,
                      int* count_dev, int* nearest_dev, int ld_nearest, void* stream);

size_t d3f_validation_pairs_workspace_bytes(int P, int ld_idx);
int d3f_validation_pairs(const float* desc, int ldd, int C, const float* score, int lds, const float* points, int ldp, int n_rows,
                         const int* row0_dev, const int* anc_dev, const int* pos_dev, int ld_idx, const int* n_dev, int P,
                         float safe_radius, int keypts_num, float det_loss_weight, float pos_margin, float neg_margin,
                         float log_scale, float* values, int* status_dev, double* sums_dev, int64_t* counts_dev, void* workspace,
                         size_t workspace_bytes, void* stream);

size_t d3f_loss_gradients_workspace_bytes(int P, int ld_idx, int C);
int d3f_loss_gradients(const float* desc, int ldd, int C, const float* score, int lds, const float* points, int ldp, int n_rows,
                       const int* row0_dev, const int* anc_dev, const int* pos_dev, int ld_idx, const int* n_dev, int P,
                       float safe_radius, int keypts_num, float det_loss_weight, float pos_margin, float neg_margin, float log_scale,
                       int contrastive, float* grad_desc, int ldg, float* grad_score, int ldgs, float* values, int* status_dev,
                       void* workspace, size_t workspace_bytes, void* stream);

size_t d3f_neighbor_transpose_workspace_bytes(int N, int K);
int d3f_neighbor_transpose(const int* idx, int N, int ld_idx, int K, const int* lens_dev, int B, int* start, int* edges, void* workspace,
                           size_t workspace_bytes, void* stream);

size_t d3f_detect_head_backward_workspace_bytes(int N, int C, int B);
int d3f_detect_head_backward(const float* x, int N, int ldx, int C, const int* idx, int ld_idx, int K, const int* lens_dev,
                             const int* include_zero_dev, int stack_group, int B, const int* start, const int* edges,
                             const float* gdesc, int ldg, const float* gscore, int ldgs, float* gx, int ldgx, void* workspace,
                             size_t workspace_bytes, void* stream);

int d3f_neighbor_transpose_qs(const int* idx, int Nq, int ld_idx, int K, const int* Nq_dev, int Ns, const int* Ns_dev, int* start,
                              int* edges, void* workspace, size_t workspace_bytes, void* stream);

size_t d3f_kpconv_backward_workspace_bytes(int Nq, int Ns, int K, int Cin, int Cout, int num_kp);
int d3f_kpconv_backward(const float* q, int Nq, const float* s, int Ns, const int* idx, int ld_idx, int K, const void* f, int ldf,
                        int Cin, const float* kp_host, int num_kp, float KP_extent, int influence, int aggregation, const float* W,
                        const float* gout, int ldg, int Cout, const int* start, const int* edges, float* gf, int ldgf, float* gW,
                        const int* Nq_dev, const int* Ns_dev, const int* q_order, int feat_bf16, void* workspace,
                        size_t workspace_bytes, void* stream);

size_t d3f_gemm_tn_workspace_bytes(int M, int Ca, int Cb);
int d3f_gemm_tn_f32(const float* A, int lda, const float* B, int ldb, int M, int Ca, int Cb, float* out, const int* M_dev,
                    void* workspace, size_t workspace_bytes, void* stream);

size_t d3f_batch_norm_workspace_bytes(int M, int C);
int d3f_batch_norm_train(const float* x, int ldx, int M, int C, const float* gamma, const float* beta, float eps, float momentum,
                         float* moving_mean, float* moving_var, const float* residual, int ldr, int leaky, float alpha, float* y, int ldy,
                         float* mean, float* rstd, const int* M_dev, void* workspace, size_t workspace_bytes, void* stream);
int d3f_batch_norm_backward(const float* x, int ldx, const float* y, int ldy, const float* gy, int ldg, int M, int C, const float* gamma,
                            const float* mean, const float* rstd, int leaky, float alpha, float* gx, int ldgx, float* ggamma,
                            float* gbeta, float* gres, int ldgr, const int* M_dev, void* workspace, size_t workspace_bytes, void* stream);

int d3f_pose_errors(const float* T_est, const float* gt, int P, int per_pair, const double* thresholds_host, double* rte_dev,
                    double* rre_deg_dev, int* flags_dev, double* meters_dev, void* stream);

int d3f_sanitize_descriptors(float* kp, int n_blocks, int K, int ld, int C, void* stream);

int d3f_matching_summary(const int* mutual_count, const int* gt_inliers, const int* gt_flag, int P, int n, const int* scene_start_host,
                         int S, const double* inlier_ratio_host, int* ratio_e8, long long* figures, void* stream);

int d3f_registration_recall(const void* T_est, int logged, const double* gt, const double* info, const int* gt_flag,
                            const int* result_flag, const int* ids, int P, int n, const int* scene_start_host, int S,
                            const double* err2_host, double* error, int* flags, long long* figures, void* stream);

size_t d3f_icp_pairs_workspace_bytes(int N_src, int B);
int d3f_icp_pairs(const void* grid, size_t grid_bytes, int N_tgt, const float* src, int N_src, const int* src_lens_dev, int B,
                  const double* init, const double* criteria_host, int max_iteration, int check_every, double* T, int* count,
                  double* sumd2, double* fitness, double* rmse, int* iterations, int* converged, int* nearest, void* workspace,
                  size_t workspace_bytes, void* stream);

#ifdef __cplusplus
}
#endif
#endif
```

Measured before the change: 1986 fragments/s.

## Sort grid-subsample voxel keys per cloud with segmented radix sort

Adds a segmented radix sort for grid subsampling, on by default and switchable off through D3F_GS_SEGMENTED=0. Each cloud gets its own tile rows and histograms, so the sort key no longer carries the batch index. This drops the batch bits from the key width and can remove a radix pass. The heads and runs kernels become templated to detect cloud boundaries from the offsets. In exchange, more histogram rows are used, extra per-tile segment lookups are added, and the kernel and host code become more complex.

```diff
diff --git a/d3feat_amd/_lib.py b/d3feat_amd/_lib.py
--- a/d3feat_amd/_lib.py
+++ b/d3feat_amd/_lib.py
@@ -29,6 +29,8 @@
     "d3f_batch_grid_subsample": (_i, [_vp, _i, _vp, _i, _f, _vp, _i, _vp, _i, _vp, _vp, _vp, _vp, _vp, _vp, _sz, _vp]),
     "d3f_batch_grid_subsample_async": (_i, [_vp, _i, _vp, _i, _f, _vp, _i, _i, _i, _vp, _vp, _vp, _sz, _vp]),
     "d3f_batch_grid_subsample_async_inplace": (_i, [_vp, _i, _vp, _i, _f, _vp, _i, _i, _vp, _vp, _vp, _sz, _vp]),
+    "d3f_grid_subsample_segmented": (_i, [_i]),
+    "d3f_radix_segment_rows": (_i, [_vp, _i, _i, _vp, _vp]),
     "d3f_stack_self_pair": (_i, [_vp, _i, _vp, _i, _vp, _vp, _vp, _vp]),
     "d3f_radius_neighbors_workspace_bytes": (_sz, [_i, _i, _i]),
     "d3f_batch_radius_neighbors": (_i, [_vp, _i, _vp, _i, _vp, _vp, _i, _f, _vp, _i, _i, _i, _vp, _vp, _sz, _vp]),
diff --git a/d3feat_amd/csrc/grid_subsample.hip b/d3feat_amd/csrc/grid_subsample.hip
--- a/d3feat_amd/csrc/grid_subsample.hip
+++ b/d3feat_amd/csrc/grid_subsample.hip
@@ -50,7 +50,7 @@
 }
 __device__ __forceinline__ void gs_prep(const unsigned* __restrict__ bbox, const int* __restrict__ offs, int B, float dl,
                                         GsElem* __restrict__ el, int* __restrict__ status, RsMeta* __restrict__ smeta,
-                                        int n_cap) {
+                                        int n_cap, int* __restrict__ row0 = nullptr) {
     __shared__ unsigned long long sCells[256];
     const int b = threadIdx.x;
     unsigned long long cells = 0ull;
@@ -87,6 +87,7 @@
         cells = c >= 1.8e19 ? 0xFFFFFFFFFFFFFFFFull : e.NX * e.NY * e.NZ;
     }
     if (!smeta) return;
+    if (row0 && b < B) row0[b] = rs_seg_row0(offs, b, min(offs[B], n_cap));
     sCells[threadIdx.x] = cells;
     __syncthreads();
     if (threadIdx.x == 0) {
@@ -103,20 +104,23 @@
             atomicOr(&status[1], D3F_ST_KEY_WIDTH);
             m.n = 0;
             m.bits = 8;
+        } else if (row0) {
+            m.bits = kb;
         }
         m.npass = (m.bits + 7) / 8;
         *smeta = m;
     }
 }
 struct GsPrepEpi {
-    const unsigned* bbox; const int* offs; int B; float dl; GsElem* el; int* status; RsMeta* smeta; int n_cap;
-    __device__ __forceinline__ void operator()() const { gs_prep(bbox, offs, B, dl, el, status, smeta, n_cap); }
+    const unsigned* bbox; const int* offs; int B; float dl; GsElem* el; int* status; RsMeta* smeta; int n_cap; int* row0;
+    __device__ __forceinline__ void operator()() const { gs_prep(bbox, offs, B, dl, el, status, smeta, n_cap, row0); }
 };
 
 __global__ void __launch_bounds__(256) gs_begin_boxed_kernel(const int* __restrict__ lens, int B, int* __restrict__ offs,
                                                              const unsigned* __restrict__ bbox, unsigned* __restrict__ counters,
                                                              int ncounters, D3fFill f0, D3fFill fmeta, float dl, GsElem* __restrict__ el,
-                                                             int* __restrict__ status, RsMeta* __restrict__ smeta, int n_cap) {
+                                                             int* __restrict__ status, RsMeta* __restrict__ smeta, int n_cap,
+                                                             int* __restrict__ row0) {
     const size_t tid = (size_t)blockIdx.x * blockDim.x + threadIdx.x, stride = (size_t)gridDim.x * blockDim.x;
     d3f_fill_words(f0, tid, stride);
     if (blockIdx.x != 0) return;
@@ -129,7 +133,7 @@
     for (int i = threadIdx.x; i < (int)fmeta.n; i += blockDim.x) fmeta.p[i] = fmeta.v;
     asm volatile("s_waitcnt vmcnt(0)" ::: "memory");
     __syncthreads();
-    gs_prep(bbox, offs, B, dl, el, status, smeta, n_cap);
+    gs_prep(bbox, offs, B, dl, el, status, smeta, n_cap, row0);
 }
 
 __global__ void __launch_bounds__(256) gs_insert_kernel(const float* __restrict__ pts, int N, const int* __restrict__ offs,
@@ -409,6 +413,16 @@
 
 #include "gs_small.h"
 
+
+__device__ __forceinline__ unsigned gs_voxel_key32(const float* __restrict__ P, int i, const GsElem& e, float dl, int kb, int& st) {
+    const float ox = e.org[0], oy = e.org[1], oz = e.org[2];
+    const unsigned NX = (unsigned)e.NX, NY = (unsigned)e.NY;
+    float cx, cy, cz;
+    st |= gs_cell(P + 3 * (size_t)i, ox, oy, oz, dl, cx, cy, cz);
+    const unsigned ix = (unsigned)cx, iy = (unsigned)cy, iz = (unsigned)cz;
+    const unsigned k = ix + NX * (iy + NY * iz);
+    return kb < 32 ? (k & ((1u << kb) - 1u)) : k;
+}
 __global__ void __launch_bounds__(RS_THREADS) gs_sortkey_kernel(const float* __restrict__ pts, const float* const* __restrict__ ptrs,
                                                                 const int* __restrict__ offs, int B,
                                                                 float dl, const GsElem* __restrict__ el,
@@ -443,14 +457,7 @@
             int b = b0;
             if (!one_cloud)
                 while (b + 1 < B && i >= sOffs[b + 1]) ++b;
-            const float ox = sEl[b].org[0], oy = sEl[b].org[1], oz = sEl[b].org[2];
-            const unsigned NX = (unsigned)sEl[b].NX, NY = (unsigned)sEl[b].NY;
-            const float* __restrict__ P = sBase[b];
-            float cx, cy, cz;
-            st |= gs_cell(P + 3 * (size_t)i, ox, oy, oz, dl, cx, cy, cz);
-            const unsigned ix = (unsigned)cx, iy = (unsigned)cy, iz = (unsigned)cz;
-            const unsigned k = ix + NX * (iy + NY * iz);
-            key[r] = (kb < 32 ? ((unsigned)b << kb) : 0u) | (kb < 32 ? (k & ((1u << kb) - 1u)) : k);
+            key[r] = (kb < 32 ? ((unsigned)b << kb) : 0u) | gs_voxel_key32(sBase[b], i, sEl[b], dl, kb, st);
             skey[i] = key[r];
             vm |= 1u << r;
         }
@@ -458,16 +465,55 @@
     if (st) atomicOr(&status[1], st);
     rs_tile_histogram(key, vm, 0, sHist, hist + (size_t)tile * 256);
 }
-
+__global__ void __launch_bounds__(RS_THREADS) gs_sortkey_seg_kernel(const float* __restrict__ pts, const float* const* __restrict__ ptrs,
+                                                                    RsSeg seg, float dl, const GsElem* __restrict__ el,
+                                                                    const RsMeta* __restrict__ smeta, unsigned* __restrict__ skey,
+                                                                    unsigned* __restrict__ hist, int* __restrict__ status) {
+    __shared__ unsigned sHist[256];
+    __shared__ GsElem sE;
+    const int n = smeta->n, kb = smeta->kb;
+    RsSegTile t;
+    if (!rs_seg_tile(seg, n, blockIdx.x, t)) return;
+    const int b = t.b;
+    if (threadIdx.x == 0) sE = el[b];
+    __syncthreads();
+    const float* __restrict__ P = ptrs ? ptrs[b] - 3 * (size_t)seg.offs[b] : pts;
+    const int w = threadIdx.x >> 6, lane = threadIdx.x & 63;
+    const int base = t.tile * RS_TILE + w * RS_WAVE_ITEMS + lane;
+    unsigned key[RS_ROUNDS], vm = 0u;
+    int st = 0;
+#pragma unroll
+    for (int r = 0; r < RS_ROUNDS; ++r) {
+        const int pos = base + r * 64;
+        key[r] = 0u;
+        if (pos < t.len) {
+            key[r] = gs_voxel_key32(P, t.lo + pos, sE, dl, kb, st);
+            skey[t.lo + pos] = key[r];
+            vm |= 1u << r;
+        }
+    }
+    if (st) atomicOr(&status[1], st);
+    rs_tile_histogram(key, vm, 0, sHist, hist + ((size_t)t.row0 + (size_t)t.tile) * 256);
+}
+
+__device__ __forceinline__ int gs_cloud_from(const int* __restrict__ offs, int B, int b0, int j) {
+    int b = b0;
+    while (b + 1 < B && j >= offs[b + 1]) ++b;
+    return b;
+}
+template <bool SEG>
 __global__ void __launch_bounds__(256) gs_heads_kernel(int N, const RsMeta* __restrict__ smeta, const unsigned* __restrict__ key0,
                                                        const unsigned* __restrict__ key1, const unsigned* __restrict__ val0,
-                                                       const unsigned* __restrict__ val1, unsigned* __restrict__ fbits) {
+                                                       const unsigned* __restrict__ val1, unsigned* __restrict__ fbits,
+                                                       const int* __restrict__ offs, int B) {
     const int j = blockIdx.x * blockDim.x + threadIdx.x;
     if (j >= min(N, smeta->n)) return;
     const unsigned* __restrict__ ks = (smeta->npass & 1) ? key1 : key0;
     const unsigned* __restrict__ vs = (smeta->npass & 1) ? val1 : val0;
     const unsigned k = ks[j];
-    if (j == 0 || ks[j - 1] != k) {
+    bool first = false;
+    if constexpr (SEG) first = offs[gs_cloud_from(offs, B, d3f_find_elem(offs, B, blockIdx.x * blockDim.x), j)] == j;
+    if (j == 0 || first || ks[j - 1] != k) {
         const unsigned i = vs[j];
         atomicOr(&fbits[i >> 5], 1u << (i & 31u));
     }
@@ -476,11 +522,12 @@
     const unsigned* fbits;
     __device__ __forceinline__ int operator()(int w) const { return __popc(fbits[w]); }
 };
+template <bool SEG>
 __global__ void __launch_bounds__(256) gs_runs_kernel(int N, const RsMeta* __restrict__ smeta, const unsigned* __restrict__ key0,
                                                       const unsigned* __restrict__ key1, const unsigned* __restrict__ val0,
                                                       const unsigned* __restrict__ val1, GsRankBits rank,
                                                       const float* __restrict__ pts, const float* const* __restrict__ ptrs,
-                                                      const int* __restrict__ offs, unsigned long long* __restrict__ vkey,
+                                                      const int* __restrict__ offs, int B, unsigned long long* __restrict__ vkey,
                                                       float* __restrict__ bary) {
     __shared__ float sx[256], sy[256], sz[256];
     __shared__ unsigned sk[256];
@@ -492,24 +539,30 @@
     const unsigned* __restrict__ vs = (smeta->npass & 1) ? val1 : val0;
     unsigned k = 0u, pi = 0u, kprev = 0u;
     float px = 0.f, py = 0.f, pz = 0.f;
+    int cbeg = 0, cend = n;
     if (j < n) {
         k = ks[j];
         pi = vs[j];
         kprev = j > 0 ? ks[j - 1] : 0u;
-        if (ptrs) {
-            const int b = smeta->kb < 32 ? (int)(k >> smeta->kb) : 0;
-            pts = ptrs[b] - 3 * (size_t)offs[b];
-        }
+        int b = 0;
+        if constexpr (SEG) {
+            b = gs_cloud_from(offs, B, d3f_find_elem(offs, B, j0), j);
+            cbeg = offs[b];
+            cend = rs_seg_begin(offs, b + 1, n);
+        } else {
+            b = smeta->kb < 32 ? (int)(k >> smeta->kb) : 0;
+        }
+        if (ptrs) pts = ptrs[b] - 3 * (size_t)offs[b];
         px = pts[3 * (size_t)pi + 0]; py = pts[3 * (size_t)pi + 1]; pz = pts[3 * (size_t)pi + 2];
     }
     sx[t] = px; sy[t] = py; sz[t] = pz;
     sk[t] = k;
     __syncthreads();
-    if (j >= n || (j != 0 && kprev == k)) return;
+    if (j >= n || (j != 0 && kprev == k && !(SEG && j == cbeg))) return;
     const int v = rank((int)pi);
     float ax = px, ay = py, az = pz;
     int c = 1;
-    const int lim = min(256, n - j0);
+    const int lim = min(256, (SEG ? cend : n) - j0);
     while (t + c < lim && sk[t + c] == k) {
         ax = __fadd_rn(ax, sx[t + c]);
         ay = __fadd_rn(ay, sy[t + c]);
@@ -517,7 +570,7 @@
         ++c;
     }
     if (t + c == 256) {
-        while (j + c < n && ks[j + c] == k) {
+        while (j + c < cend && ks[j + c] == k) {
             const size_t q = vs[j + c];
             ax = __fadd_rn(ax, pts[3 * q + 0]);
             ay = __fadd_rn(ay, pts[3 * q + 1]);
@@ -633,8 +686,8 @@
     bytes += 6 * d3f_align((size_t)L.bucket_total * sizeof(int));
     bytes += d3f_align((n / GS_TILE + B + 8) * sizeof(int));
     bytes += 2 * d3f_align(d3f_scan_base_ints(N) * sizeof(int)) + d3f_align((4 + D3F_NCHAIN * (size_t)B) * sizeof(unsigned));
-    bytes += d3f_align(rs_hist_words(N) * sizeof(unsigned)) + d3f_align((n / 32 + 2) * sizeof(unsigned)) +
-             d3f_align(3 * n * sizeof(float)) + d3f_align(sizeof(RsMeta));
+    bytes += d3f_align(rs_hist_words(N, B) * sizeof(unsigned)) + d3f_align((n / 32 + 2) * sizeof(unsigned)) +
+             d3f_align(3 * n * sizeof(float)) + d3f_align(sizeof(RsMeta)) + d3f_align(B * sizeof(int));
     bytes += d3f_align(7 * (size_t)B * (n < 16384 ? n : 16384) * sizeof(float)) + 256 + 2 * d3f_align(B * sizeof(int));
     return bytes + 4096;
 }
@@ -709,6 +762,7 @@
     unsigned* fbits;
     float* bary;
     RsMeta* smeta;
+    int* seg_row0;
 
     bool carve(void* workspace, size_t workspace_bytes, int N, int B, int keys) {
         L = gs_layout(N, B, keys);
@@ -748,10 +802,11 @@
         A.tsum = ar.take<int>(n / GS_TILE + B + 8);
         vbase = ar.take<int>(d3f_scan_base_ints(N));
         sbase = ar.take<int>(d3f_scan_base_ints(N));
-        rs_hist = ar.take<unsigned>(rs_hist_words(N));
+        rs_hist = ar.take<unsigned>(rs_hist_words(N, B));
         fbits = ar.take<unsigned>(n / 32 + 2);
         bary = ar.take<float>(3 * n);
         smeta = ar.take<RsMeta>(1);
+        seg_row0 = ar.take<int>(B);
         A.vkey = vkey; A.moffs = moffs; A.offs = offs; A.el = el;
         return ar.ok;
     }
@@ -774,11 +829,40 @@
     return D3F_OK;
 }
 
+static std::atomic<int> gs_segmented{-1};
+extern "C" int d3f_grid_subsample_segmented(int on) {
+    int cur = gs_segmented.load(std::memory_order_relaxed);
+    if (cur < 0) {
+        const char* e = std::getenv("D3F_GS_SEGMENTED");
+        cur = (e && e[0] == '0' && e[1] == '\0') ? 0 : 1;
+        gs_segmented.store(cur, std::memory_order_relaxed);
+    }
+    if (on >= 0) gs_segmented.store(on ? 1 : 0, std::memory_order_relaxed);
+    return cur;
+}
+extern "C" int d3f_radix_segment_rows(const int* lens, int B, int n_cap, int* tiles, int* row0) {
+    if (!lens || !tiles || !row0 || B < 1 || B > D3F_MAX_BATCH || n_cap < 1 || n_cap > (1 << 30)) return D3F_ERR_ARG;
+    int offs[D3F_MAX_BATCH + 1];
+    offs[0] = 0;
+    for (int b = 0; b < B; ++b) {
+        if (lens[b] < 0 || lens[b] > (1 << 30) - offs[b]) return D3F_ERR_ARG;
+        offs[b + 1] = offs[b] + lens[b];
+    }
+    const int n = offs[B] < n_cap ? offs[B] : n_cap;
+    for (int b = 0; b < B; ++b) {
+        tiles[b] = rs_seg_tiles(offs, b, n);
+        row0[b] = rs_seg_row0(offs, b, n);
+    }
+    return rs_seg_rows(n_cap, B);
+}
+
 static int gs_run_sort(const GsCall& C, const GsWork& W, int elem_cap) {
     const int N = C.N, B = C.B;
     const size_t n = (size_t)N;
     hipStream_t stream = C.stream;
     int rc;
+    const bool segmented = d3f_grid_subsample_segmented(-1) != 0;
+    int* const row0 = segmented ? W.seg_row0 : nullptr;
     const D3fFill none{nullptr, 0ull, 0u};
     const D3fFill fill_bits{W.fbits, (unsigned long long)(n / 32 + 2), 0u};
     const D3fFill fill_meta{(unsigned*)W.meta, (unsigned long long)(B + 2), 0u};
@@ -786,28 +870,42 @@
         long long blocks = (long long)(fill_bits.n / 4 / 256) + 1;
         if (blocks > 1024) blocks = 1024;
         gs_begin_boxed_kernel<<<(int)blocks, 256, 0, stream>>>(C.lens_dev, B, W.offs, C.bbox_in, W.counters, W.ncounters, fill_bits,
-                                                               fill_meta, C.dl, W.el, W.meta, W.smeta, N);
+                                                               fill_meta, C.dl, W.el, W.meta, W.smeta, N, row0);
         D3F_LAUNCH_CHECK();
     } else {
         if ((rc = d3f_begin_launch(C.lens_dev, B, W.offs, W.bbox, W.counters, W.ncounters, fill_bits, fill_meta, none, none,
                                    stream)) != D3F_OK)
             return rc;
-        GsPrepEpi prep{W.bbox, W.offs, B, C.dl, W.el, W.meta, W.smeta, N};
+        GsPrepEpi prep{W.bbox, W.offs, B, C.dl, W.el, W.meta, W.smeta, N, row0};
         if ((rc = d3f_bbox_launch_t(C.points, W.offs, B, N, W.bbox, W.counters, prep, stream, C.ptrs)) != D3F_OK) return rc;
     }
     const int nblk = d3f_cdiv(N, 256);
     unsigned *key0 = (unsigned*)W.slot, *key1 = (unsigned*)W.pnext, *val0 = (unsigned*)W.pvid, *val1 = (unsigned*)W.sorted;
-    gs_sortkey_kernel<<<rs_tiles(N), RS_THREADS, 0, stream>>>(C.points, C.ptrs, W.offs, B, C.dl, W.el, W.smeta, key0, W.rs_hist,
-                                                              W.meta);
-    D3F_LAUNCH_CHECK();
-    if ((rc = rs_sort_launch(W.smeta, N, key0, key1, val0, val1, W.rs_hist, stream)) != D3F_OK) return rc;
-    gs_heads_kernel<<<nblk, 256, 0, stream>>>(N, W.smeta, key0, key1, val0, val1, W.fbits);
-    D3F_LAUNCH_CHECK();
     const GsRankBits rank{W.fbits, W.vscan, W.vbase};
     GsMoffsEpi<GsRankBits> mepi{W.offs, B, rank, W.meta, W.moffs, C.sub_lens_dev, C.status_dev, C.M_cap, elem_cap};
-    if ((rc = d3f_scan_fold_launch(GsBitsIn{W.fbits}, N / 32 + 1, nullptr, W.vscan, W.vbase, W.counters + 1, mepi, stream)) != D3F_OK)
-        return rc;
-    gs_runs_kernel<<<nblk, 256, 0, stream>>>(N, W.smeta, key0, key1, val0, val1, rank, C.points, C.ptrs, W.offs, W.vkey, W.bary);
+    if (segmented) {
+        const RsSeg seg{W.offs, W.seg_row0, B};
+        gs_sortkey_seg_kernel<<<rs_seg_rows(N, B), RS_THREADS, 0, stream>>>(C.points, C.ptrs, seg, C.dl, W.el, W.smeta, key0, W.rs_hist, W.meta);
+        D3F_LAUNCH_CHECK();
+        if ((rc = rs_sort_launch(W.smeta, N, key0, key1, val0, val1, W.rs_hist, stream, &seg)) != D3F_OK) return rc;
+        gs_heads_kernel<true><<<nblk, 256, 0, stream>>>(N, W.smeta, key0, key1, val0, val1, W.fbits, W.offs, B);
+        D3F_LAUNCH_CHECK();
+        if ((rc = d3f_scan_fold_launch(GsBitsIn{W.fbits}, N / 32 + 1, nullptr, W.vscan, W.vbase, W.counters + 1, mepi, stream)) != D3F_OK)
+            return rc;
+        gs_runs_kernel<true><<<nblk, 256, 0, stream>>>(N, W.smeta, key0, key1, val0, val1, rank, C.points, C.ptrs, W.offs, B, W.vkey,
+                                                       W.bary);
+    } else {
+        gs_sortkey_kernel<<<rs_tiles(N), RS_THREADS, 0, stream>>>(C.points, C.ptrs, W.offs, B, C.dl, W.el, W.smeta, key0, W.rs_hist,
+                                                                  W.meta);
+        D3F_LAUNCH_CHECK();
+        if ((rc = rs_sort_launch(W.smeta, N, key0, key1, val0, val1, W.rs_hist, stream)) != D3F_OK) return rc;
+        gs_heads_kernel<false><<<nblk, 256, 0, stream>>>(N, W.smeta, key0, key1, val0, val1, W.fbits, W.offs, B);
+        D3F_LAUNCH_CHECK();
+        if ((rc = d3f_scan_fold_launch(GsBitsIn{W.fbits}, N / 32 + 1, nullptr, W.vscan, W.vbase, W.counters + 1, mepi, stream)) != D3F_OK)
+            return rc;
+        gs_runs_kernel<false><<<nblk, 256, 0, stream>>>(N, W.smeta, key0, key1, val0, val1, rank, C.points, C.ptrs, W.offs, B, W.vkey,
+                                                        W.bary);
+    }
     D3F_LAUNCH_CHECK();
     const int M = N < C.M_cap ? N : C.M_cap;
     if ((rc = gs_order_launch(W, B, elem_cap, stream)) != D3F_OK) return rc;
diff --git a/d3feat_amd/csrc/radix_sort.h b/d3feat_amd/csrc/radix_sort.h
--- a/d3feat_amd/csrc/radix_sort.h
+++ b/d3feat_amd/csrc/radix_sort.h
@@ -16,8 +16,25 @@
 };
 
 #define RS_SCATTER_LDS_BYTES ((2 * RS_WAVES * 256 + 256 + 16 + 2 * RS_TILE) * 4)
+#define RS_SCATTER_SEG_LDS_BYTES ((RS_WAVES * 256 + 256 + 16 + 2 * RS_TILE) * 4)
 static inline int rs_tiles(int n_cap) { return d3f_cdiv(n_cap > 0 ? n_cap : 1, RS_TILE); }
-static inline size_t rs_hist_words(int n_cap) { return (size_t)rs_tiles(n_cap) * 256; }
+static inline size_t rs_hist_words(int n_cap, int segments = 0) { return ((size_t)rs_tiles(n_cap) + (size_t)segments) * 256; }
+
+struct RsSeg {
+    const int* offs;
+    const int* row0;
+    int B;
+};
+__host__ __device__ inline int rs_seg_begin(const int* offs, int b, int n) { return offs[b] < n ? offs[b] : n; }
+__host__ __device__ inline int rs_seg_tiles(const int* offs, int b, int n) {
+    return (rs_seg_begin(offs, b + 1, n) - rs_seg_begin(offs, b, n) + RS_TILE - 1) / RS_TILE;
+}
+__host__ __device__ inline int rs_seg_row0(const int* offs, int b, int n) {
+    int r = 0;
+    for (int j = 0; j < b; ++j) r += rs_seg_tiles(offs, j, n);
+    return r;
+}
+static inline int rs_seg_rows(int n_cap, int segments) { return rs_tiles(n_cap) + segments; }
 
 #ifdef __HIPCC__
 __device__ __forceinline__ void rs_tile_histogram(const unsigned (&key)[RS_ROUNDS], unsigned valid_mask, int shift,
@@ -57,6 +74,140 @@
         }
     }
     return loc;
+}
+
+__device__ __forceinline__ void rs_hist_tile(int lo, int len, int tile, int shift, const unsigned* __restrict__ src,
+                                             unsigned* __restrict__ sHist, unsigned* __restrict__ hist) {
+    const int w = threadIdx.x >> 6, lane = threadIdx.x & 63;
+    const int base = tile * RS_TILE + w * RS_WAVE_ITEMS + lane;
+    unsigned key[RS_ROUNDS], vm = 0u;
+#pragma unroll
+    for (int r = 0; r < RS_ROUNDS; ++r) {
+        const int pos = base + r * 64;
+        key[r] = 0u;
+        if (pos < len) { key[r] = src[lo + pos]; vm |= 1u << r; }
+    }
+    rs_tile_histogram(key, vm, shift, sHist, hist + (size_t)tile * 256);
+}
+
+template <bool OVERLAY>
+__device__ __forceinline__ void rs_scatter_tile(unsigned* rs_lds, int lo, int len, int tile, int live, int pass,
+                                                const unsigned* __restrict__ ksrc, const unsigned* __restrict__ vsrc,
+                                                unsigned* __restrict__ kdst, unsigned* __restrict__ vdst,
+                                                const unsigned* __restrict__ hist) {
+    unsigned (*sCnt)[256] = (unsigned (*)[256])rs_lds;
+    unsigned* sBase = rs_lds + (OVERLAY ? 1 : 2) * RS_WAVES * 256;
+    unsigned* sScan = sBase + 256;
+    unsigned* sKey = sScan + 16;
+    unsigned* sVal = sKey + RS_TILE;
+    unsigned (*sPart)[256] = (unsigned (*)[256])(OVERLAY ? sKey : rs_lds + RS_WAVES * 256);
+    const int tid = threadIdx.x, w = tid >> 6, lane = tid & 63;
+    const int shift = pass * 8;
+
+    const int base = tile * RS_TILE + w * RS_WAVE_ITEMS + lane;
+    unsigned key[RS_ROUNDS], val[RS_ROUNDS];
+#pragma unroll
+    for (int r = 0; r < RS_ROUNDS; ++r) {
+        const int pos = base + r * 64;
+        key[r] = 0u;
+        val[r] = (unsigned)(lo + pos);
+        if (pos < len) {
+            key[r] = ksrc[lo + pos];
+            if (pass > 0) val[r] = vsrc[lo + pos];
+        }
+    }
+    {
+        uint4 bef = make_uint4(0u, 0u, 0u, 0u), tot = make_uint4(0u, 0u, 0u, 0u);
+        const uint4* __restrict__ rows = (const uint4*)hist + lane;
+        int t = w;
+        constexpr int U = OVERLAY ? 4 : 8;
+        for (; t + (U - 1) * RS_WAVES < live; t += U * RS_WAVES) {
+            uint4 v[U];
+#pragma unroll
+            for (int u = 0; u < U; ++u) v[u] = rows[(size_t)(t + u * RS_WAVES) * 64];
+#pragma unroll
+            for (int u = 0; u < U; ++u) {
+                tot.x += v[u].x; tot.y += v[u].y; tot.z += v[u].z; tot.w += v[u].w;
+                if (t + u * RS_WAVES < tile) { bef.x += v[u].x; bef.y += v[u].y; bef.z += v[u].z; bef.w += v[u].w; }
+            }
+        }
+        for (; t < live; t += RS_WAVES) {
+            const uint4 v = rows[(size_t)t * 64];
+            tot.x += v.x; tot.y += v.y; tot.z += v.z; tot.w += v.w;
+            if (t < tile) { bef.x += v.x; bef.y += v.y; bef.z += v.z; bef.w += v.w; }
+        }
+        ((uint4*)sCnt[w])[lane] = tot;
+        ((uint4*)sPart[w])[lane] = bef;
+    }
+    __syncthreads();
+    {
+        unsigned total = 0u, before = 0u;
+        if (tid < 256) {
+#pragma unroll
+            for (int q = 0; q < RS_WAVES; ++q) { total += sCnt[q][tid]; before += sPart[q][tid]; }
+        }
+        const unsigned x = d3f_wave_incl_scan(total);
+        if (lane == 63) sScan[w] = x;
+        __syncthreads();
+#pragma unroll
+        for (int q = 0; q < RS_WAVES; ++q)
+            if (tid < 256) sCnt[q][tid] = 0u;
+        unsigned wb = 0u;
+#pragma unroll
+        for (int q = 0; q < 4; ++q) wb += (q < w) ? sScan[q] : 0u;
+        if (tid < 256) sBase[tid] = (unsigned)lo + wb + x - total + before;
+        __syncthreads();
+    }
+    unsigned rank[RS_ROUNDS];
+    volatile unsigned* myCnt = sCnt[w];
+#pragma unroll
+    for (int r = 0; r < RS_ROUNDS; ++r) {
+        const bool valid = (base + r * 64) < len;
+        const unsigned dg = (key[r] >> shift) & 255u;
+        unsigned long long peers = __ballot(valid);
+#pragma unroll
+        for (int bit = 0; bit < 8; ++bit) {
+            const bool one = (dg >> bit) & 1u;
+            const unsigned long long m = __ballot(one);
+            peers &= one ? m : ~m;
+        }
+        rank[r] = 0u;
+        if (valid) {
+            const unsigned prev = myCnt[dg];
+            const unsigned below = (unsigned)__popcll(peers & d3f_lanemask_lt());
+            rank[r] = prev + below;
+            __builtin_amdgcn_wave_barrier();
+            if (below == 0u) myCnt[dg] = prev + (unsigned)__popcll(peers);
+        }
+        __builtin_amdgcn_wave_barrier();
+    }
+    __syncthreads();
+    {
+        const unsigned loc = rs_wave_bases<RS_WAVES>(sCnt, sScan);
+        if (tid < 256) sBase[tid] -= loc;
+    }
+    __syncthreads();
+#pragma unroll
+    for (int r = 0; r < RS_ROUNDS; ++r) {
+        if ((base + r * 64) < len) {
+            const unsigned dg = (key[r] >> shift) & 255u;
+            const unsigned pl = myCnt[dg] + rank[r];
+            sKey[pl] = key[r];
+            sVal[pl] = val[r];
+        }
+    }
+    __syncthreads();
+    const int tile_n = min(RS_TILE, len - tile * RS_TILE);
+#pragma unroll
+    for (int r = 0; r < RS_ROUNDS; ++r) {
+        const int pl = r * RS_THREADS + tid;
+        if (pl < tile_n) {
+            const unsigned k = sKey[pl];
+            const unsigned dest = sBase[(k >> shift) & 255u] + (unsigned)pl;
+            kdst[dest] = k;
+            vdst[dest] = sVal[pl];
+        }
+    }
 }
 
 __global__ void __launch_bounds__(RS_THREADS) rs_hist_kernel(const RsMeta* __restrict__ meta, int pass,
@@ -68,17 +219,7 @@
     if (pass >= meta->npass) return;
     const int tile = blockIdx.x;
     if ((long long)tile * RS_TILE >= (long long)n) return;
-    const unsigned* __restrict__ src = (pass & 1) ? key1 : key0;
-    const int w = threadIdx.x >> 6, lane = threadIdx.x & 63;
-    const int base = tile * RS_TILE + w * RS_WAVE_ITEMS + lane;
-    unsigned key[RS_ROUNDS], vm = 0u;
-#pragma unroll
-    for (int r = 0; r < RS_ROUNDS; ++r) {
-        const int pos = base + r * 64;
-        key[r] = 0u;
-        if (pos < n) { key[r] = src[pos]; vm |= 1u << r; }
-    }
-    rs_tile_histogram(key, vm, pass * 8, sHist, hist + (size_t)tile * 256);
+    rs_hist_tile(0, n, tile, pass * 8, (pass & 1) ? key1 : key0, sHist, hist);
 }
 
 __global__ void __launch_bounds__(RS_THREADS) rs_scatter_kernel(const RsMeta* __restrict__ meta, int pass,
@@ -86,133 +227,68 @@
                                                                 unsigned* __restrict__ val0, unsigned* __restrict__ val1,
                                                                 const unsigned* __restrict__ hist) {
     extern __shared__ __attribute__((aligned(16))) unsigned rs_lds[];
-    unsigned (*sCnt)[256] = (unsigned (*)[256])rs_lds;
-    unsigned (*sPart)[256] = (unsigned (*)[256])(rs_lds + RS_WAVES * 256);
-    unsigned* sBase = rs_lds + 2 * RS_WAVES * 256;
-    unsigned* sScan = sBase + 256;
-    unsigned* sKey = sScan + 16;
-    unsigned* sVal = sKey + RS_TILE;
     const int n = meta->n;
     if (pass >= meta->npass) return;
     const int tile = blockIdx.x;
     if ((long long)tile * RS_TILE >= (long long)n) return;
     const int live = (n + RS_TILE - 1) / RS_TILE;
-    const unsigned* __restrict__ ksrc = (pass & 1) ? key1 : key0;
-    const unsigned* __restrict__ vsrc = (pass & 1) ? val1 : val0;
-    unsigned* __restrict__ kdst = (pass & 1) ? key0 : key1;
-    unsigned* __restrict__ vdst = (pass & 1) ? val0 : val1;
-    const int tid = threadIdx.x, w = tid >> 6, lane = tid & 63;
-    const int shift = pass * 8;
-
-    const int base = tile * RS_TILE + w * RS_WAVE_ITEMS + lane;
-    unsigned key[RS_ROUNDS], val[RS_ROUNDS];
-#pragma unroll
-    for (int r = 0; r < RS_ROUNDS; ++r) {
-        const int pos = base + r * 64;
-        key[r] = 0u;
-        val[r] = (unsigned)pos;
-        if (pos < n) {
-            key[r] = ksrc[pos];
-            if (pass > 0) val[r] = vsrc[pos];
-        }
-    }
-    {
-        uint4 bef = make_uint4(0u, 0u, 0u, 0u), tot = make_uint4(0u, 0u, 0u, 0u);
-        const uint4* __restrict__ rows = (const uint4*)hist + lane;
-        int t = w;
-        for (; t + 7 * RS_WAVES < live; t += 8 * RS_WAVES) {
-            uint4 v[8];
-#pragma unroll
-            for (int u = 0; u < 8; ++u) v[u] = rows[(size_t)(t + u * RS_WAVES) * 64];
-#pragma unroll
-            for (int u = 0; u < 8; ++u) {
-                tot.x += v[u].x; tot.y += v[u].y; tot.z += v[u].z; tot.w += v[u].w;
-                if (t + u * RS_WAVES < tile) { bef.x += v[u].x; bef.y += v[u].y; bef.z += v[u].z; bef.w += v[u].w; }
+    rs_scatter_tile<false>(rs_lds, 0, n, tile, live, pass, (pass & 1) ? key1 : key0, (pass & 1) ? val1 : val0, (pass & 1) ? key0 : key1,
+                           (pass & 1) ? val0 : val1, hist);
+}
+
+struct RsSegTile { int b, lo, len, tile, live, row0; };
+__device__ __forceinline__ bool rs_seg_tile(const RsSeg& seg, int n, int row, RsSegTile& t) {
+    const int b = d3f_find_elem(seg.row0, seg.B, row);
+    t.b = b;
+    t.lo = rs_seg_begin(seg.offs, b, n);
+    t.len = rs_seg_begin(seg.offs, b + 1, n) - t.lo;
+    t.live = (t.len + RS_TILE - 1) / RS_TILE;
+    t.row0 = seg.row0[b];
+    t.tile = row - t.row0;
+    return t.tile < t.live;
+}
+
+__global__ void __launch_bounds__(RS_THREADS) rs_hist_seg_kernel(const RsMeta* __restrict__ meta, int pass, RsSeg seg,
+                                                                 const unsigned* __restrict__ key0,
+                                                                 const unsigned* __restrict__ key1,
+                                                                 unsigned* __restrict__ hist) {
+    __shared__ unsigned sHist[256];
+    if (pass >= meta->npass) return;
+    RsSegTile t;
+    if (!rs_seg_tile(seg, meta->n, blockIdx.x, t)) return;
+    rs_hist_tile(t.lo, t.len, t.tile, pass * 8, (pass & 1) ? key1 : key0, sHist, hist + (size_t)t.row0 * 256);
+}
+
+__global__ void __launch_bounds__(RS_THREADS) __attribute__((amdgpu_waves_per_eu(4, 4)))
+rs_scatter_seg_kernel(const RsMeta* __restrict__ meta, int pass, RsSeg seg, unsigned* __restrict__ key0, unsigned* __restrict__ key1,
+                      unsigned* __restrict__ val0, unsigned* __restrict__ val1, const unsigned* __restrict__ hist) {
+    extern __shared__ __attribute__((aligned(16))) unsigned rs_lds[];
+    if (pass >= meta->npass) return;
+    RsSegTile t;
+    if (!rs_seg_tile(seg, meta->n, blockIdx.x, t)) return;
+    rs_scatter_tile<true>(rs_lds, t.lo, t.len, t.tile, t.live, pass, (pass & 1) ? key1 : key0, (pass & 1) ? val1 : val0,
+                          (pass & 1) ? key0 : key1, (pass & 1) ? val0 : val1, hist + (size_t)t.row0 * 256);
+}
+#endif
+
+static inline int rs_sort_launch(const RsMeta* meta, int n_cap, unsigned* key0, unsigned* key1, unsigned* val0, unsigned* val1,
+                                 unsigned* hist, hipStream_t stream, const RsSeg* seg = nullptr) {
+    const int tiles = rs_tiles(n_cap);
+    if (seg && seg->offs) {
+        static std::atomic<unsigned long long> seg_lds_done{0ull};
+        const void* const seg_fns[] = {(const void*)rs_scatter_seg_kernel};
+        if (d3f_opt_in_lds(seg_lds_done, seg_fns, RS_SCATTER_SEG_LDS_BYTES) != D3F_OK) return D3F_ERR_HIP;
+        const int rows = rs_seg_rows(n_cap, seg->B);
+        for (int p = 0; p < RS_MAX_PASSES; ++p) {
+            if (p > 0) {
+                rs_hist_seg_kernel<<<rows, RS_THREADS, 0, stream>>>(meta, p, *seg, key0, key1, hist);
+                D3F_LAUNCH_CHECK();
             }
-        }
-        for (; t < live; t += RS_WAVES) {
-            const uint4 v = rows[(size_t)t * 64];
-            tot.x += v.x; tot.y += v.y; tot.z += v.z; tot.w += v.w;
-            if (t < tile) { bef.x += v.x; bef.y += v.y; bef.z += v.z; bef.w += v.w; }
-        }
-        ((uint4*)sCnt[w])[lane] = tot;
-        ((uint4*)sPart[w])[lane] = bef;
-    }
-    __syncthreads();
-    {
-        unsigned total = 0u, before = 0u;
-        if (tid < 256) {
-#pragma unroll
-            for (int q = 0; q < RS_WAVES; ++q) { total += sCnt[q][tid]; before += sPart[q][tid]; }
-        }
-        const unsigned x = d3f_wave_incl_scan(total);
-        if (lane == 63) sScan[w] = x;
-        __syncthreads();
-#pragma unroll
-        for (int q = 0; q < RS_WAVES; ++q)
-            if (tid < 256) sCnt[q][tid] = 0u;
-        unsigned wb = 0u;
-#pragma unroll
-        for (int q = 0; q < 4; ++q) wb += (q < w) ? sScan[q] : 0u;
-        if (tid < 256) sBase[tid] = wb + x - total + before;
-        __syncthreads();
-    }
-    unsigned rank[RS_ROUNDS];
-    volatile unsigned* myCnt = sCnt[w];
-#pragma unroll
-    for (int r = 0; r < RS_ROUNDS; ++r) {
-        const bool valid = (base + r * 64) < n;
-        const unsigned dg = (key[r] >> shift) & 255u;
-        unsigned long long peers = __ballot(valid);
-#pragma unroll
-        for (int bit = 0; bit < 8; ++bit) {
-            const bool one = (dg >> bit) & 1u;
-            const unsigned long long m = __ballot(one);
-            peers &= one ? m : ~m;
-        }
-        rank[r] = 0u;
-        if (valid) {
-            const unsigned prev = myCnt[dg];
-            const unsigned below = (unsigned)__popcll(peers & d3f_lanemask_lt());
-            rank[r] = prev + below;
-            __builtin_amdgcn_wave_barrier();
-            if (below == 0u) myCnt[dg] = prev + (unsigned)__popcll(peers);
-        }
-        __builtin_amdgcn_wave_barrier();
-    }
-    __syncthreads();
-    {
-        const unsigned loc = rs_wave_bases<RS_WAVES>(sCnt, sScan);
-        if (tid < 256) sBase[tid] -= loc;
-    }
-    __syncthreads();
-#pragma unroll
-    for (int r = 0; r < RS_ROUNDS; ++r) {
-        if ((base + r * 64) < n) {
-            const unsigned dg = (key[r] >> shift) & 255u;
-            const unsigned pl = myCnt[dg] + rank[r];
-            sKey[pl] = key[r];
-            sVal[pl] = val[r];
-        }
-    }
-    __syncthreads();
-    const int tile_n = min(RS_TILE, n - tile * RS_TILE);
-#pragma unroll
-    for (int r = 0; r < RS_ROUNDS; ++r) {
-        const int pl = r * RS_THREADS + tid;
-        if (pl < tile_n) {
-            const unsigned k = sKey[pl];
-            const unsigned dest = sBase[(k >> shift) & 255u] + (unsigned)pl;
-            kdst[dest] = k;
-            vdst[dest] = sVal[pl];
-        }
-    }
-}
-#endif
-
-static inline int rs_sort_launch(const RsMeta* meta, int n_cap, unsigned* key0, unsigned* key1, unsigned* val0, unsigned* val1,
-                                 unsigned* hist, hipStream_t stream) {
-    const int tiles = rs_tiles(n_cap);
+            rs_scatter_seg_kernel<<<rows, RS_THREADS, RS_SCATTER_SEG_LDS_BYTES, stream>>>(meta, p, *seg, key0, key1, val0, val1, hist);
+            D3F_LAUNCH_CHECK();
+        }
+        return D3F_OK;
+    }
     static std::atomic<unsigned long long> lds_done{0ull};
     const void* const fns[] = {(const void*)rs_scatter_kernel};
     if (d3f_opt_in_lds(lds_done, fns, RS_SCATTER_LDS_BYTES) != D3F_OK) return D3F_ERR_HIP;
diff --git a/include/d3feat_amd.h b/include/d3feat_amd.h
--- a/include/d3feat_amd.h
+++ b/include/d3feat_amd.h
@@ -47,6 +47,8 @@
 int d3f_batch_grid_subsample_async_inplace(const float* const* clouds_dev, int N_cap, const int* lens_dev, int B, float dl,
                                            float* sub_points, int M_cap, int elem_cap, int* sub_lens_dev, int* status_dev,
                                            void* workspace, size_t workspace_bytes, void* stream);
+int d3f_grid_subsample_segmented(int on);
+int d3f_radix_segment_rows(const int* lens, int B, int n_cap, int* tiles, int* row0);
 
 int d3f_stack_self_pair(const float* pts, int M_cap, const int* lens_in_dev, int B, float* out, int* lens_out_dev,
                         int* total_dev, void* stream);
```

Measured after the change: 1999 fragments/s (median of 6 runs). About the same (+0.7%).
